# mjq11302010044/TATT

Hardware: AMD Instinct MI355X
Metric: LR images/s (train fwd+bwd+clip+Adam) at 16x64->32x128 (higher is better)
Workload: dtype fp32 (split-bf16 MFMA operands in conv3 / conv3-wgrad / conv9 / tokgemm / gru-wgrad / query-GRU recurrence and dW_hh / TP-layer backward)

## Files before the change

include/tatt_hip.h:

```cpp
#ifndef TATT_HIP_H
#define TATT_HIP_H

#ifdef __cplusplus
extern "C" {
#endif

typedef struct ihipStream_t* hipStream_t;


int tatt_gemm(const float* A, long sam, long sak, const float* A2, long sa2m, long sa2k, int K1,
              const float* B, long sbk, long sbn, const float* bias, float* C, long scm, long scn,
              int M, int N, int K, int Z, long bsA, long bsA2, long bsB, long bsC, long bsBias,
              float alpha, float beta, int act, int splitk, float* ws, float* rowsum, hipStream_t st);

int tatt_conv2d_fwd(const float* x, long xsn, long xsh, long xsw, long xsc, const float* wpacked,
                    const float* bias, float* y, long ldy, int Bn, int H, int W, int Cin, int Cout,
                    int KH, int KW, int act, float beta, int splitk, float* ws, hipStream_t st);

int tatt_conv2d_fwd_partials(const float* x, long xsn, long xsh, long xsw, long xsc, const float* wpacked, int Bn, int H,
                             int W, int Cin, int Cout, int KH, int KW, int splitk, float* ws, int* splits, hipStream_t st);

int tatt_conv2d_wgrad(const float* x, long xsn, long xsh, long xsw, long xsc, const float* dy,
                      long lddy, float* dw_oihw, int Bn, int H, int W, int Cin, int Cout, int KH,
                      int KW, float beta, int splitk, float* ws, hipStream_t st);

int tatt_repack_conv_weight(const float* w_oihw, float* out, int Cout, int Cin, int KH, int KW,
                            int mode, hipStream_t st);
int tatt_repack_words(int Cout, int Cin, int KH, int KW, int mode);
int tatt_repack_conv_weight_batch(const float* const* ws, float* const* outs, const int* dims, int n, hipStream_t st);

int tatt_gru_wgrad_sb(const float* dgi, const float* dgh, const float* x, const float* xb, const float* hprev,
                      float* ws1, float* ws2, int M, int G, hipStream_t st);

int tatt_splitk_reduce(const float* partial, float* C, int M, int N, int S, int remap_cin, int remap_taps,
                       float beta, float* vec, int vec_len, hipStream_t st);
int tatt_reduce_defer(int on, hipStream_t st);
int tatt_reduce_flush(hipStream_t st);

int tatt_conv3_c64_fwd_t(const float* x, const float* wt, const float* bias, float* y, int B, int H, int W, int Cin,
                         int Cout, int act, float beta, hipStream_t st);
int tatt_conv3_c64_fwd_ws16(const float* x, const float* wl, const float* bias, float* y, int B, int H, int W,
                            int Cout, int act, float beta, hipStream_t st);
int tatt_conv3_c64_fwd_ws16_bn(const float* x, const float* wl, const float* bias, float* y, int B, int H, int W,
                               int Cout, int act, float beta, const float* in_scale, const float* in_shift, int in_act,
                               double* stats, hipStream_t st);
int tatt_conv3_c64_fwd_sb(const float* x, int cin_total, int ci0, const float* wl, const float* bias, float* y, int B, int H,
                          int W, int Cout, int act, float beta, const float* in_scale, const float* in_shift, int in_act,
                          double* stats, hipStream_t st);
int tatt_conv3_c64_dgrad_bn_sb(const float* x, const float* x2, const float* in_scale, const float* in_scale2,
                               const float* in_shift, const float* wl, float* y, int B, int H, int W, const float* ep_x,
                               const float* ep_mean, const float* ep_rstd, const float* ep_gamma, const float* ep_beta,
                               int ep_act, double* stats, hipStream_t st);
int tatt_conv3_sb_generation(int gen);
int tatt_conv3_sb_packing(int B, int H, int W, int cin_total, int Cout, int act, int ep_act);
int tatt_conv3_sb_route(int B, int H, int W, int cin_total, int Cout, int act, int ep_act);
int tatt_conv3_c64_wgrad_partial(const float* x, const float* dy, float* part, float* pdb, int B, int H, int W,
                                 int Cin, int Cout, int G, hipStream_t st);
int tatt_conv3_c64_wgrad_partial_sb(const float* x, const float* dy, float* part, float* pdb, int B, int H, int W,
                                    int Cin, int Cout, int G, hipStream_t st);
int tatt_conv3_wgrad_sb_generation(int gen);
int tatt_conv3_wgrad_sb_route(int B, int H, int W, int Cin, int Cout);

int tatt_conv9_c64_to_c4(const float* x, const float* wpacked, const float* bias, float* y, int B, int H, int W,
                         int C, hipStream_t st);
int tatt_conv9_c64_to_c4_mfma(const float* x, const float* wt, const float* bias, float* y, int B, int H, int W,
                              hipStream_t st);
int tatt_conv9_c64_to_c4_sb(const float* x, const float* wt, const float* bias, float* y, int B, int H, int W,
                            hipStream_t st);
int tatt_conv9_c4_to_c64(const float* in, const float* wp, const float* bias, float* out, int B, int H, int W, int act,
                         hipStream_t st);
int tatt_conv9_c4_to_c64_sb(const float* in, const float* wp, const float* bias, float* out, int B, int H, int W, int act,
                            hipStream_t st);
int tatt_conv9_c64_c4_wgrad(const float* x, const float* dy, float* dw, float* part, int B, int H, int W,
                            hipStream_t st);
int tatt_conv9_c4_c64_wgrad(const float* x, const float* dy, float* dw, float* part, int B, int H, int W,
                            hipStream_t st);
int tatt_conv9_c64_c4_wgrad_sb(const float* x, const float* dy, float* dw, float* part, int B, int H, int W,
                               hipStream_t st);
int tatt_conv9_c4_c64_wgrad_sb(const float* x, const float* dy, float* dw, float* part, int B, int H, int W,
                               hipStream_t st);


int tatt_colsum(const float* X, long ld, int M, int C, float* out, float scale, float beta,
                double* ws, hipStream_t st);

int tatt_bn_stats(const float* X, long ld, int M, int C, float eps, float momentum, float* mean,
                  float* rstd, float* running_mean, float* running_var, double* ws, hipStream_t st);
int tatt_bn_stats_finish(const double* part, int G, int C, int M, float eps, float momentum, const float* gamma,
                         const float* beta, float* mean, float* rstd, float* running_mean, float* running_var, float* scale,
                         float* shift, hipStream_t st);
int tatt_bn_rstd(const float* var, float* rstd, int C, float eps, hipStream_t st);
int tatt_bn_apply(const float* X, long ldx, float* Y, long ldy, int M, int C, const float* mean,
                  const float* rstd, const float* gamma, const float* beta, int act, hipStream_t st);
int tatt_bn_bwd(const float* X, long ldx, const float* dY, long lddy, float* dX, long lddx, int M, int C,
                const float* mean, const float* rstd, const float* gamma, const float* beta, int act,
                int training, float* dgamma, float* dbeta, float* sums, double* ws, hipStream_t st);
int tatt_bn_bwd_groups(int M);
int tatt_bn_bwd_partials(const float* X, long ldx, const float* dY, long lddy, int M, int C, const float* mean,
                         const float* rstd, const float* gamma, const float* beta, int act, double* part, hipStream_t st);
int tatt_bn_bwd_finish(const double* part, int G, int C, int M, const float* mean, const float* rstd, const float* gamma,
                       float* dgamma, float* dbeta, float* coef, hipStream_t st);
int tatt_bn_bwd_affine(const float* X, const float* dU, float* dX, int M, int C, const float* coef, hipStream_t st);

int tatt_ln_fwd(const float* A, const float* Bres, float* Y, float* stats, int M, int C,
                const float* gamma, const float* beta, float eps, int mode, float pdrop,
                const unsigned long long* seed, unsigned site, hipStream_t st);
int tatt_ln_bwd(const float* A, const float* Bres, const float* dY, const float* stats, float* dX, float* dB, int M,
                int C, const float* gamma, float* dgamma, float* dbeta, float* part, double* ws, float eps, int mode,
                float pdrop, const unsigned long long* seed, unsigned site, hipStream_t st);


int tatt_prelu_fwd(const float* x, float* y, const float* alpha, long n, hipStream_t st);
int tatt_prelu_bwd(const float* x, const float* dy, float* dx, const float* alpha, long n, float* part,
                   hipStream_t st);
int tatt_act_fwd(const float* x, float* y, long n, int act, hipStream_t st);
int tatt_act_bwd(const float* ref, const float* dy, float* dx, long n, int act, int from_output,
                 hipStream_t st);
int tatt_axpby(const float* a, const float* b, float* y, float alpha, float beta, long n, hipStream_t st);
int tatt_add_n(const float* const* srcs, int n, float* y, long numel, hipStream_t st);
int tatt_add_rowbcast(const float* a, const float* b, float* y, long rows, int C, long period,
                      hipStream_t st);
int tatt_pixel_shuffle_fwd(const float* in, float* out, int B, int H, int W, int C, int act,
                           hipStream_t st);
int tatt_pixel_shuffle_bwd(const float* in, const float* dout, float* din, int B, int H, int W, int C,
                           int act, hipStream_t st);
int tatt_maxpool_fwd(const float* in, float* out, int B, int H, int W, int C, int kh, int kw, int sh, int sw,
                     int ph, int pw, hipStream_t st);
int tatt_maxpool_bwd(const float* in, const float* dout, float* din, int B, int H, int W, int C, int kh,
                     int kw, int sh, int sw, int ph, int pw, hipStream_t st);
int tatt_dropout(const float* x, float* y, long n, float p, const unsigned long long* seed, unsigned site,
                 hipStream_t st);
int tatt_bump_seed(unsigned long long* seed, unsigned long long* snap, hipStream_t st);
int tatt_stamp(unsigned long long* out, hipStream_t st);
int tatt_copy4d(const float* src, float* dst, int n0, int n1, int n2, int n3, long s0, long s1, long s2,
                long s3, long d0, long d1, long d2, long d3, float beta, hipStream_t st);


int tatt_l2norm(const float* g, long n, float* out, double* ws, hipStream_t st);
int tatt_adam_step(float* p, const float* g, float* m, float* v, long n, float lr, float b1, float b2,
                   float eps, const float* gnorm, float max_norm, float gscale, const long long* step,
                   hipStream_t st);


int tatt_gru32_fwd(const float* gi, const float* whh_f, const float* bhh_f, const float* whh_r,
// ... 293 lines not shown
```

tatt_amd/csrc/conv3.hip:

```cpp
#include "common.h"
#include <mutex>
#include <stdlib.h>
#include <type_traits>

#define C3_PX 64
#define C3_HW 66

struct Conv3P {
    const float* x; const float* w; const float* bias; float* y;
    int B, H, W, Cin, Cout, act;
    float beta;
    const float* in_scale; const float* in_shift; int in_act;
    double* stats;
};
template <int CK>
struct C5 {
    static constexpr int XP = CK + 4;
    static constexpr int HALO = 3 * C3_HW * XP;
    static constexpr int WT = 64 * XP;
    static constexpr int LDS = (2 * HALO + 2 * WT) * 4;
    static constexpr int Q4 = CK / 4;
    static constexpr int SLICE = 22 * Q4;
    static constexpr int WF4 = 64 * Q4;
};
// ... 239 lines not shown
        acc[1] = (f32x4){0.f, 0.f, 0.f, 0.f};
        f32x4 va[3][2];
        f32x4 hq = (f32x4){0.f, 0.f, 0.f, 0.f};
#define W16_AOFF(l, m) ((((l) >> 2) / 3 * C3_HW + ((l) >> 2) % 3 + 16 * (m)) * W16_XP + 16 * ((l) & 3))
#define W16_LD(l) va[(l) % 3][0] = *reinterpret_cast<const f32x4*>(Xs + W16_AOFF(l, 0)); \
                  va[(l) % 3][1] = *reinterpret_cast<const f32x4*>(Xs + W16_AOFF(l, 1));
        W16_LD(0) W16_LD(1)
#pragma unroll
        for (int l = 0; l < 36; ++l) {
            if (l % 5 == 0 && has_next) hq = halo_load(nn, nh, nw0, t + 512 * (l / 5));
            if (l + 2 < 36) { W16_LD(l + 2) }
            __builtin_amdgcn_sched_barrier(0);
#pragma unroll
            for (int u = 0; u < 4; ++u) {
                acc[0] = __builtin_amdgcn_mfma_f32_16x16x4f32(va[l % 3][0][u], wq[l][u], acc[0], 0, 0, 0);
                acc[1] = __builtin_amdgcn_mfma_f32_16x16x4f32(va[l % 3][1][u], wq[l][u], acc[1], 0, 0, 0);
            }
            __builtin_amdgcn_sched_barrier(0);
            if (l % 5 == 4 && has_next) halo_store(XsN, t + 512 * (l / 5), hq);
        }
        {
            const long rowbase = ((long)n * p.H + h) * p.W + w0 + pxh * 32 + 4 * (lane >> 4);
#pragma unroll
            for (int m = 0; m < 2; ++m)
#pragma unroll
                for (int r = 0; r < 4; ++r) {
                    float* dst = p.y + (rowbase + 16 * m + r) * p.Cout + co0 + (lane & 15);
                    float v = acc[m][r] + bj;
                    if (p.beta != 0.f) v += p.beta * *dst;
                    v = apply_act(v, p.act);
                    *dst = v;
                    st_s += v; st_q += v * v;
                }
        }
        if (!has_next) break;
        __syncthreads();
        pt = npt_next; n = nn; h = nh; w0 = nw0;
        xbuf ^= 1;
    }
    if (p.stats) {
        st_s += __shfl_xor(st_s, 16, 64); st_s += __shfl_xor(st_s, 32, 64);
        st_q += __shfl_xor(st_q, 16, 64); st_q += __shfl_xor(st_q, 32, 64);
        if (lane < 16) { st_red[pxh][0][cq * 16 + lane] = st_s; st_red[pxh][1][cq * 16 + lane] = st_q; }
        __syncthreads();
        if (t < 128) p.stats[(long)blockIdx.x * 128 + t] = (double)st_red[0][t >> 6][t & 63] + (double)st_red[1][t >> 6][t & 63];
    }
}

TATT_API int tatt_conv3_c64_fwd_ws16_bn(const float* x, const float* wl, const float* bias, float* y, int B, int H, int W,
                                        int Cout, int act, float beta, const float* in_scale, const float* in_shift, int in_act,
                                        double* stats, hipStream_t st);
TATT_API int tatt_conv3_c64_fwd_ws16(const float* x, const float* wl, const float* bias, float* y, int B, int H, int W,
                                     int Cout, int act, float beta, hipStream_t st) {
    return tatt_conv3_c64_fwd_ws16_bn(x, wl, bias, y, B, H, W, Cout, act, beta, nullptr, nullptr, 0, nullptr, st);
}
TATT_API int tatt_conv3_c64_fwd_ws16_bn(const float* x, const float* wl, const float* bias, float* y, int B, int H, int W,
                                        int Cout, int act, float beta, const float* in_scale, const float* in_shift, int in_act,
                                        double* stats, hipStream_t st) {
    if (Cout % 64 || W % C3_PX) return 1;
    if (stats && (Cout != 64 || act != ACT_NONE || beta != 0.f)) return 2;
    if (in_scale && (!in_shift || in_act == ACT_TANH)) return 3;
    Conv3P p = {x, wl, bias, y, B, H, W, 64, Cout, act, beta, in_scale, in_shift, in_act, stats};
    static TattPerDevice attr_once;
    tatt_per_device(attr_once, [&] {
        (void)hipFuncSetAttribute(reinterpret_cast<const void*>(conv3_c64_ws16_kernel), hipFuncAttributeMaxDynamicSharedMemorySize, W16_LDS);
    });
    const int cob = Cout / 64, npt = B * H * (W / C3_PX);
    int per = 256 / cob;
    if (per > npt) per = npt;
    hipLaunchKernelGGL(conv3_c64_ws16_kernel, dim3(per * cob), dim3(512), W16_LDS, st, p);
    return LAUNCH_CHECK();
}

typedef __bf16 bf16x8 __attribute__((ext_vector_type(8)));
typedef __bf16 bf16x2 __attribute__((ext_vector_type(2)));
typedef float f32x2 __attribute__((ext_vector_type(2)));
#define SB_PW 40
#define SB_IMG (3 * C3_HW * SB_PW)
#define SB_LDS (4 * SB_IMG * 4)
struct Conv3SB {
    Conv3P c; int cin_total, ci0;
    const float* x2; const float* in_scale2;
    const float* ep_x; const float* ep_mean; const float* ep_rstd; const float* ep_gamma; const float* ep_beta; int ep_act;
};
__device__ __forceinline__ void sb_split(f32x4 v, uint2& hi, uint2& lo) {
    const bf16x2 h0 = __builtin_convertvector((f32x2){v[0], v[1]}, bf16x2), h1 = __builtin_convertvector((f32x2){v[2], v[3]}, bf16x2);
    const unsigned u0 = __builtin_bit_cast(unsigned, h0), u1 = __builtin_bit_cast(unsigned, h1);
    const float r0 = v[0] - __builtin_bit_cast(float, u0 << 16), r1 = v[1] - __builtin_bit_cast(float, u0 & 0xffff0000u);
    const float r2 = v[2] - __builtin_bit_cast(float, u1 << 16), r3 = v[3] - __builtin_bit_cast(float, u1 & 0xffff0000u);
    const bf16x2 l0 = __builtin_convertvector((f32x2){r0, r1}, bf16x2), l1 = __builtin_convertvector((f32x2){r2, r3}, bf16x2);
    hi = make_uint2(u0, u1);
    lo = make_uint2(__builtin_bit_cast(unsigned, l0), __builtin_bit_cast(unsigned, l1));
}
template <bool IN2, bool EPBN>
__global__ __launch_bounds__(512, 1) void conv3_c64_sb_kernel(Conv3SB q) {
    const Conv3P& p = q.c;
    extern __shared__ __attribute__((aligned(16))) unsigned smem_u[];
    const int t = threadIdx.x, lane = t & 63, wave = t >> 6;
    const int cq = wave & 3, pxh = wave >> 2;
    const int segs = p.W / C3_PX, cob = p.Cout / 64;
    const int npt = p.B * p.H * segs;
    const int stride = gridDim.x / cob;
    int cb = blockIdx.x % cob, pt = blockIdx.x / cob;
    if (gridDim.x % 8 == 0 && 8 % cob == 0 && stride % (8 / cob) == 0) {
        const int x = blockIdx.x & 7, m = blockIdx.x >> 3, xg = 8 / cob;
        cb = x % cob;
        pt = (x / cob) * (stride / xg) + m;
    }
    __shared__ float st_red[2][2][64];
    if (pt >= npt) {
        if (p.stats && t < 128) p.stats[(long)blockIdx.x * 128 + t] = 0.0;
        return;
    }
    const int co0 = cb * 64 + cq * 16;
    f32x4 isc = (f32x4){1.f, 1.f, 1.f, 1.f}, ish = (f32x4){0.f, 0.f, 0.f, 0.f};
    if (p.in_scale) {
        isc = *reinterpret_cast<const f32x4*>(p.in_scale + 4 * (t & 15));
        ish = *reinterpret_cast<const f32x4*>(p.in_shift + 4 * (t & 15));
    }
    f32x4 isc2 = (f32x4){0.f, 0.f, 0.f, 0.f};
    if (IN2) isc2 = *reinterpret_cast<const f32x4*>(q.in_scale2 + 4 * (t & 15));
    float ep_mu = 0.f, ep_rs = 0.f, ep_g = 0.f, ep_b = 0.f;
    if (EPBN) {
        const int c = co0 + (lane & 15);
        ep_mu = q.ep_mean[c]; ep_rs = q.ep_rstd[c]; ep_g = q.ep_gamma[c]; ep_b = q.ep_beta[c];
    }
    float st_s = 0.f, st_q = 0.f;
    f32x4 wq[36];
    {
        const f32x4* wsrc = reinterpret_cast<const f32x4*>(p.w) + (long)(cb * 4 + cq) * 36 * 64 + lane;
#pragma unroll
        for (int k = 0; k < 36; ++k) wq[k] = wsrc[k * 64];
    }
    auto decode = [&](int tile, int& n, int& h, int& w0) {
        const int seg = tile % segs; tile /= segs;
        h = tile % p.H; n = tile / p.H; w0 = seg * C3_PX;
    };
    auto halo_load = [&](int n, int h, int w0, int idx) -> f32x4 {
        const int pix = idx >> 4, r = pix / C3_HW, px = pix - r * C3_HW;
        const int hh = h + r - 1, ww = w0 + px - 1;
        f32x4 v = (f32x4){0.f, 0.f, 0.f, 0.f};
        if (idx < 3 * C3_HW * 16 && hh >= 0 && hh < p.H && ww >= 0 && ww < p.W) {
            v = *reinterpret_cast<const f32x4*>(p.x + (((long)n * p.H + hh) * p.W + ww) * q.cin_total + q.ci0 + 4 * (idx & 15));
            if (IN2) {
                const f32x4 v2 = *reinterpret_cast<const f32x4*>(q.x2 + (((long)n * p.H + hh) * p.W + ww) * 64 + 4 * (idx & 15));
#pragma unroll
                for (int e = 0; e < 4; ++e) v[e] = fmaf(v[e], isc[e], fmaf(v2[e], isc2[e], ish[e]));
            } else if (p.in_scale) {
#pragma unroll
                for (int e = 0; e < 4; ++e) {
                    const float u = fmaf(v[e], isc[e], ish[e]);
                    v[e] = p.in_act == ACT_MISH ? mish_f(u) : (p.in_act == ACT_RELU ? fmaxf(u, 0.f) : u);
                }
            }
        }
        return v;
    };
    auto halo_store = [&](unsigned* Xs, int idx, f32x4 v) {
        if (idx < 3 * C3_HW * 16) {
            uint2 hi, lo;
            sb_split(v, hi, lo);
            unsigned* d = Xs + (idx >> 4) * SB_PW + 2 * (idx & 15);
            *reinterpret_cast<uint2*>(d) = hi;
            *reinterpret_cast<uint2*>(d + SB_IMG) = lo;
        }
    };
    int n, h, w0;
    decode(pt, n, h, w0);
    {
        f32x4 hp[7];
#pragma unroll
        for (int k = 0; k < 7; ++k) hp[k] = halo_load(n, h, w0, t + 512 * k);
#pragma unroll
        for (int k = 0; k < 7; ++k) halo_store(smem_u, t + 512 * k, hp[k]);
    }
// ... 282 lines not shown
        unsigned nnorg, nnte;
        decode(pt + 2 * stride, nnorg, nnte);
#pragma unroll
        for (int st = 0; st < 18; ++st) {
            if (st + 1 < 18) { S3_LD(st + 1) }
            if (FIRST && st % 2 == 0 && st / 2 + 3 < 9) w_issue(st / 2 + 3);
            __builtin_amdgcn_sched_barrier(0);
            const bf16x8 wh = __builtin_bit_cast(bf16x8, wq[2 * st]), wl = __builtin_bit_cast(bf16x8, wq[2 * st + 1]);
            const bf16x8 b0h = __builtin_bit_cast(bf16x8, vb[st % 2][0]), b0l = __builtin_bit_cast(bf16x8, vb[st % 2][1]);
            const bf16x8 b1h = __builtin_bit_cast(bf16x8, vb[st % 2][2]), b1l = __builtin_bit_cast(bf16x8, vb[st % 2][3]);
            accM[0] = __builtin_amdgcn_mfma_f32_32x32x16_bf16(wh, b0h, accM[0], 0, 0, 0);
            accM[1] = __builtin_amdgcn_mfma_f32_32x32x16_bf16(wh, b1h, accM[1], 0, 0, 0);
            accC[0] = __builtin_amdgcn_mfma_f32_32x32x16_bf16(wl, b0h, accC[0], 0, 0, 0);
            accC[1] = __builtin_amdgcn_mfma_f32_32x32x16_bf16(wl, b1h, accC[1], 0, 0, 0);
            accC[0] = __builtin_amdgcn_mfma_f32_32x32x16_bf16(wh, b0l, accC[0], 0, 0, 0);
            accC[1] = __builtin_amdgcn_mfma_f32_32x32x16_bf16(wh, b1l, accC[1], 0, 0, 0);
            if (st % 2 == 1 && st / 2 < S3_NIT) {
                halo_put(imgN, nte, st / 2);
                halo_issue1(nnorg, nnte, had_next && pt + 2 * stride < npt, st / 2);
                S3_INTERLEAVE(INMODE == 1 ? 14 : 8)
            }
            if (st % 4 == 2 && st / 4 < S3_NEP) { epilogue(epi_pending, st / 4); S3_INTERLEAVE(8) }
            if (st % 4 == 0 && st > 0 && st / 4 - 1 < S3_NEP) epi_request(org, st / 4 - 1);
            __builtin_amdgcn_sched_barrier(0);
        }
#if S2_STAMP
        { const unsigned long long now = __builtin_amdgcn_s_memtime();
          if (tix == 0) ts[3] = now; else if (tix == 1) ts[6] = now; else if (tix == 2) ts[9] = now; }
#endif
        has_next = had_next && pt + 2 * stride < npt;
        {
            unsigned* xw = XCH + xbuf * S2_XCH + (kh * 64 + lj) * S2_XP + 32 * coh + 4 * kb;
#pragma unroll
            for (int pp = 0; pp < 2; ++pp)
#pragma unroll
                for (int g = 0; g < 4; ++g) {
                    f32x4 v;
#pragma unroll
                    for (int r = 0; r < 4; ++r) v[r] = accM[pp][4 * g + r] + accC[pp][4 * g + r];
                    *reinterpret_cast<f32x4*>(xw + 32 * pp * S2_XP + 8 * g) = v;
                }
        }
        eorg = org; ebuf = xbuf; epi_pending = true;
#if S2_STAMP
        { const unsigned long long now = __builtin_amdgcn_s_memtime();
          if (tix == 0) ts[4] = now; else if (tix == 1) ts[7] = now; else if (tix == 2) ts[10] = now; }
        ++tix;
#endif
        __syncthreads();
        if (had_next) { pt += stride; org = norg; te = nte; norg = nnorg; nte = nnte; xbuf ^= 1; }
    };
    tile_body(std::true_type{});
    while (had_next) tile_body(std::false_type{});
    S2_STAMP_AT(11)
#pragma unroll
    for (int e = 0; e < S3_NEP; ++e) epilogue(true, e);
    S2_STAMP_AT(12)
#if S2_STAMP
    ts[31] = wall_clock64();
    if (lane == 0 && sbuf) {
#pragma unroll
        for (int i = 0; i < 32; ++i) sbuf[(blockIdx.x * 8 + wave) * 32 + i] = ts[i];
    }
#endif
    if (p.stats) {
#pragma unroll
        for (int r = 0; r < 4; ++r) {
            st_s[r] += __shfl_xor(st_s[r], 16, 64); st_s[r] += __shfl_xor(st_s[r], 32, 64);
            st_q[r] += __shfl_xor(st_q[r], 16, 64); st_q[r] += __shfl_xor(st_q[r], 32, 64);
        }
        if (lane < 16) {
#pragma unroll
            for (int r = 0; r < 4; ++r) { st_red[wave][0][ec4 + r] = st_s[r]; st_red[wave][1][ec4 + r] = st_q[r]; }
        }
        __syncthreads();
        if (t < 128) {
            double a = 0.0;
#pragma unroll
            for (int w = 0; w < 4; ++w) a += (double)st_red[w][t >> 6][t & 63];
            p.stats[(long)blockIdx.x * 128 + t] = a;
        }
    }
}
template <int INMODE, bool EPBN>
__global__ __launch_bounds__(512, 2) void conv3_c64_sb4_kernel(Conv3SB q) {
    const Conv3P& p = q.c;
    extern __shared__ __attribute__((aligned(16))) unsigned smem_u[];
    unsigned* const XCH = smem_u + 4 * S3_IMG;
    const unsigned t = threadIdx.x, lane = t & 63, wave = t >> 6;
    const unsigned W = p.W, H = p.H, tws = (W + 15) / 16, ths = H / 4, cob = p.Cout / 64;
    const unsigned npt = p.B * ths * tws;
    const unsigned stride = gridDim.x / cob;
    unsigned cb = blockIdx.x % cob, pt = blockIdx.x / cob;
    if (gridDim.x % 8 == 0 && 8 % cob == 0 && stride % (8 / cob) == 0) {
        const unsigned x = blockIdx.x & 7, m = blockIdx.x >> 3, xg = 8 / cob;
        cb = x % cob;
        pt = (x / cob) * (stride / xg) + m;
    }
    __shared__ float st_red[4][2][64];
    __shared__ __attribute__((aligned(16))) float cst[7][64];
    __shared__ __attribute__((aligned(16))) float cbias[64];
    if (pt >= npt) {
        if (p.stats && t < 128) p.stats[(long)blockIdx.x * 128 + t] = 0.0;
        return;
    }
    const unsigned ntile = (npt - pt + stride - 1) / stride;
    auto decode = [&](unsigned tile, unsigned& org, unsigned& te) {
        const unsigned tw = tile % tws; tile /= tws;
        const unsigned th = tile % ths, n = tile / ths;
        org = (n * H + th * 4) * W + tw * 16;
        const unsigned cin = min(18u, W - tw * 16 + 1);
        te = (th == 0 ? 1u : 0u) | (th == ths - 1 ? 2u : 0u) | (tw == 0 ? 4u : 0u) | (cin << 8);
    };
    if (wave >= 4) {
        const unsigned h = t - 256;
        const unsigned npix = p.B * H * W;
        const __amdgpu_buffer_rsrc_t rs_x = __builtin_amdgcn_make_buffer_rsrc(const_cast<float*>(p.x), 0, npix * q.cin_total * 4, 0x00020000);
        const __amdgpu_buffer_rsrc_t rs_x2 = __builtin_amdgcn_make_buffer_rsrc(const_cast<float*>(INMODE == 2 ? q.x2 : p.x), 0, npix * 256, 0x00020000);
        const __amdgpu_buffer_rsrc_t rs_y = __builtin_amdgcn_make_buffer_rsrc(p.y, 0, npix * p.Cout * 4, 0x00020000);
        const __amdgpu_buffer_rsrc_t rs_e = __builtin_amdgcn_make_buffer_rsrc(const_cast<float*>(EPBN ? q.ep_x : p.y), 0, npix * (EPBN ? 64 : p.Cout) * 4, 0x00020000);
        const bool in_relu = p.in_act == ACT_RELU;
        const unsigned xps = q.cin_total * 4, yps = p.Cout * 4, eps_ = EPBN ? 256u : yps;
        unsigned boff[S3_NIT], poff[S3_NIT], edge[2] = {0, 0}, colk[2] = {0, 0};
#pragma unroll
        for (int k = 0; k < S3_NIT; ++k) {
            const unsigned pix = (h >> 4) + 16 * k, r = pix / S2_HW, c = pix - r * S2_HW;
            boff[k] = (unsigned)(((int)r - 1) * (int)W + (int)c - 1) * xps + (q.ci0 + 4 * (h & 15)) * 4;
            poff[k] = r * S3_RP + c * SB_PW + 2 * (h & 15);
            edge[k >> 2] |= ((r == 0 ? 1u : 0u) | (r == 5 ? 2u : 0u) | (c == 0 ? 4u : 0u) | (pix >= S2_NPX ? 8u : 0u)) << (8 * (k & 3));
            colk[k >> 2] |= c << (8 * (k & 3));
        }
        auto outside = [&](int k, unsigned te) -> bool {
            return (((edge[k >> 2] >> (8 * (k & 3))) & (te | 8u) & 15u) != 0) || (((colk[k >> 2] >> (8 * (k & 3))) & 255u) >= (te >> 8));
        };
        f32x4 hp[S3_NIT], hp2[S3_NIT];
        auto halo_issue = [&](unsigned tile, bool valid) {
            unsigned org, te;
            decode(tile, org, te);
#if S2_DEBUG
            if (s2_wrep & 4) valid = false;
#endif
#pragma unroll
            for (int k = 0; k < S3_NIT; ++k) {
                const unsigned a = (org * xps + boff[k]) | (outside(k, te) ? S2_OOB : (valid ? 0u : S2_OOB));
                hp[k] = s2_ld(rs_x, a);
                if (INMODE == 2) hp2[k] = s2_ld(rs_x2, a);
            }
        };
        auto halo_put = [&](unsigned* img, unsigned tile) {
            unsigned org, te;
            decode(tile, org, te);
            f32x4 isc, ish, isc2;
            if (INMODE != 0) { isc = *reinterpret_cast<const f32x4*>(&cst[0][4 * (h & 15)]); ish = *reinterpret_cast<const f32x4*>(&cst[1][4 * (h & 15)]); }
            if (INMODE == 2) isc2 = *reinterpret_cast<const f32x4*>(&cst[2][4 * (h & 15)]);
#pragma unroll
            for (int k = 0; k < S3_NIT; ++k) {
                const bool ok = !outside(k, te);
                f32x4 v = hp[k];
                if (INMODE == 2) {
#pragma unroll
                    for (int e = 0; e < 4; ++e) v[e] = fmaf(v[e], isc[e], fmaf(hp2[k][e], isc2[e], ish[e]));
                } else if (INMODE == 1) {
#pragma unroll
                    for (int e = 0; e < 4; ++e) v[e] = mish_f(fmaf(v[e], isc[e], ish[e]));
                } else if (INMODE == 3) {
#pragma unroll
                    for (int e = 0; e < 4; ++e) {
                        const float u = fmaf(v[e], isc[e], ish[e]);
                        v[e] = in_relu ? fmaxf(u, 0.f) : u;
                    }
                }
                if (INMODE != 0) {
#pragma unroll
                    for (int e = 0; e < 4; ++e) v[e] = ok ? v[e] : 0.f;
                }
                if (k < S3_NIT - 1 || h < S2_NPX * 16 - 256 * (S3_NIT - 1)) {
                    uint2 hi, lo;
                    sb_split(v, hi, lo);
                    unsigned* d = img + poff[k];
                    *reinterpret_cast<uint2*>(d) = hi;
                    *reinterpret_cast<uint2*>(d + S3_IMG) = lo;
                }
            }
        };
        halo_issue(pt, true);
        if (h < 64) {
            cbias[h] = p.bias ? p.bias[cb * 64 + h] : 0.f;
            if (INMODE != 0) { cst[0][h] = p.in_scale[h]; cst[1][h] = p.in_shift[h]; }
            if (INMODE == 2) cst[2][h] = q.in_scale2[h];
            if (EPBN) { cst[3][h] = q.ep_mean[h]; cst[4][h] = q.ep_rstd[h]; cst[5][h] = q.ep_gamma[h]; cst[6][h] = q.ep_beta[h]; }
        }
        __syncthreads();
        halo_put(smem_u, pt);
        halo_issue(pt + stride, ntile > 1);
        __syncthreads();
        const bool use_beta = p.beta != 0.f, out_relu = p.act == ACT_RELU;
        const bool ep_mish = q.ep_act == ACT_MISH, ep_relu = q.ep_act == ACT_RELU;
        const unsigned ecol = h >> 4, ec4 = 4 * (h & 15);
        f32x4 epx[S3_NEP], st_s = (f32x4){0.f, 0.f, 0.f, 0.f}, st_q = st_s;
        auto epi_request = [&](unsigned tile) {
            unsigned org, te;
            decode(tile, org, te);
            const bool in_map = ecol + 1 < (te >> 8);
#pragma unroll
            for (int e = 0; e < S3_NEP; ++e)
                epx[e] = s2_ld(rs_e, ((org + e * W + ecol) * eps_ + (cb * 64 + ec4) * 4) | (((EPBN || use_beta) && in_map) ? 0u : S2_OOB));
        };
        auto epilogue = [&](unsigned tile, unsigned xb) {
            unsigned org, te;
            decode(tile, org, te);
            const f32x4 bj = *reinterpret_cast<const f32x4*>(&cbias[ec4]);
            const bool in_map = ecol + 1 < (te >> 8);
            f32x4 ep_mu, ep_rs, ep_g, ep_b;
            if (EPBN) {
                ep_mu = *reinterpret_cast<const f32x4*>(&cst[3][ec4]); ep_rs = *reinterpret_cast<const f32x4*>(&cst[4][ec4]);
                ep_g = *reinterpret_cast<const f32x4*>(&cst[5][ec4]); ep_b = *reinterpret_cast<const f32x4*>(&cst[6][ec4]);
            }
#pragma unroll
            for (int e = 0; e < S3_NEP; ++e) {
                const unsigned* X = XCH + xb * S2_XCH + ((h >> 4) + 16 * e) * S2_XP + ec4;
                const f32x4 v0 = *reinterpret_cast<const f32x4*>(X), v1 = *reinterpret_cast<const f32x4*>(X + 64 * S2_XP);
                f32x4 v;
#pragma unroll
                for (int r = 0; r < 4; ++r) {
                    v[r] = (v0[r] + v1[r]) + bj[r];
                    if (EPBN) {
                        const float xh = (epx[e][r] - ep_mu[r]) * ep_rs[r], u = fmaf(ep_g[r], xh, ep_b[r]);
                        const float g = ep_mish ? mish_grad_f(u) : 1.f;
                        v[r] *= ep_relu ? (u > 0.f ? 1.f : 0.f) : g;
                        v[r] = in_map ? v[r] : 0.f;
                        st_s[r] += v[r]; st_q[r] += v[r] * xh;
                    } else {
                        v[r] = fmaf(p.beta, epx[e][r], v[r]);
                        v[r] = out_relu ? fmaxf(v[r], 0.f) : v[r];
                        v[r] = in_map ? v[r] : 0.f;
                        st_s[r] += v[r]; st_q[r] += v[r] * v[r];
                    }
                }
#if S2_DEBUG
                if (s2_wrep & 8) continue;
#endif
                __builtin_amdgcn_raw_buffer_store_b128(__builtin_bit_cast(u32x4_s2, v), rs_y, ((org + e * W + ecol) * yps + (cb * 64 + ec4) * 4) | (in_map ? 0u : S2_OOB), 0, 0);
            }
        };
        for (unsigned i = 0; i < ntile; ++i) {
            const unsigned tile = pt + i * stride;
#if S2_DEBUG
            if (s2_wrep & 1) { __syncthreads(); continue; }
#endif
#if S2_DEBUG
            if (!(s2_wrep & 32))
#endif
            if (i > 0) epilogue(tile - stride, (i - 1) & 1);
#if S2_DEBUG
            if (!(s2_wrep & 16))
#endif
            if (i + 1 < ntile) halo_put(smem_u + ((i + 1) & 1) * 2 * S3_IMG, tile + stride);
            halo_issue(tile + 2 * stride, i + 2 < ntile);
            epi_request(tile);
            __syncthreads();
        }
        epilogue(pt + (ntile - 1) * stride, (ntile - 1) & 1);
        if (p.stats) {
#pragma unroll
            for (int r = 0; r < 4; ++r) {
                st_s[r] += __shfl_xor(st_s[r], 16, 64); st_s[r] += __shfl_xor(st_s[r], 32, 64);
                st_q[r] += __shfl_xor(st_q[r], 16, 64); st_q[r] += __shfl_xor(st_q[r], 32, 64);
            }
            if (lane < 16) {
#pragma unroll
                for (int r = 0; r < 4; ++r) { st_red[wave - 4][0][ec4 + r] = st_s[r]; st_red[wave - 4][1][ec4 + r] = st_q[r]; }
            }
        }
        __syncthreads();
        if (p.stats && h < 128) {
            double a = 0.0;
#pragma unroll
            for (int w = 0; w < 4; ++w) a += (double)st_red[w][h >> 6][h & 63];
            p.stats[(long)blockIdx.x * 128 + h] = a;
        }
        return;
    }
    const unsigned coh = wave & 1, kh = wave >> 1, lj = lane & 31, kb = lane >> 5;
    f32x4 wq[36];
    {
        const f32x4* const wsrc = reinterpret_cast<const f32x4*>(p.w) + (cb * 2 + coh) * 72 * 64 + lane;
#pragma unroll
        for (int tap = 0; tap < 9; ++tap)
#pragma unroll
            for (int f = 0; f < 4; ++f) wq[4 * tap + f] = wsrc[((tap * 2 + kh) * 4 + f) * 64];
    }
    const unsigned bbase = (lj >> 4) * S3_RP + (lj & 15) * SB_PW + 16 * kh + 4 * kb;
    __syncthreads();
    __syncthreads();
    for (unsigned i = 0; i < ntile; ++i) {
#if S2_DEBUG
        if (s2_wrep & 2) { __syncthreads(); continue; }
#endif
        const unsigned* Xs = smem_u + (i & 1) * 2 * S3_IMG + bbase;
        f32x16_s3 acc[2];
#pragma unroll
        for (int pp = 0; pp < 2; ++pp)
#pragma unroll
            for (int v = 0; v < 16; ++v) acc[pp][v] = 0.f;
        f32x4 vb[2][4];
        S3_LD(0)
#pragma unroll
        for (int st = 0; st < 18; ++st) {
            if (st + 1 < 18) { S3_LD(st + 1) }
            __builtin_amdgcn_sched_barrier(0);
            const bf16x8 wh = __builtin_bit_cast(bf16x8, wq[2 * st]), wl = __builtin_bit_cast(bf16x8, wq[2 * st + 1]);
            const bf16x8 b0h = __builtin_bit_cast(bf16x8, vb[st % 2][0]), b0l = __builtin_bit_cast(bf16x8, vb[st % 2][1]);
            const bf16x8 b1h = __builtin_bit_cast(bf16x8, vb[st % 2][2]), b1l = __builtin_bit_cast(bf16x8, vb[st % 2][3]);
            acc[0] = __builtin_amdgcn_mfma_f32_32x32x16_bf16(wh, b0h, acc[0], 0, 0, 0);
            acc[1] = __builtin_amdgcn_mfma_f32_32x32x16_bf16(wh, b1h, acc[1], 0, 0, 0);
            acc[0] = __builtin_amdgcn_mfma_f32_32x32x16_bf16(wl, b0h, acc[0], 0, 0, 0);
            acc[1] = __builtin_amdgcn_mfma_f32_32x32x16_bf16(wl, b1h, acc[1], 0, 0, 0);
            acc[0] = __builtin_amdgcn_mfma_f32_32x32x16_bf16(wh, b0l, acc[0], 0, 0, 0);
            acc[1] = __builtin_amdgcn_mfma_f32_32x32x16_bf16(wh, b1l, acc[1], 0, 0, 0);
            __builtin_amdgcn_sched_barrier(0);
        }
        unsigned* xw = XCH + (i & 1) * S2_XCH + (kh * 64 + lj) * S2_XP + 32 * coh + 4 * kb;
#pragma unroll
        for (int pp = 0; pp < 2; ++pp)
#pragma unroll
            for (int g = 0; g < 4; ++g) {
                f32x4 v;
#pragma unroll
                for (int r = 0; r < 4; ++r) v[r] = acc[pp][4 * g + r];
                *reinterpret_cast<f32x4*>(xw + 32 * pp * S2_XP + 8 * g) = v;
            }
        __syncthreads();
    }
    __syncthreads();
}
static int conv3_sb_generation = 4;
TATT_API int tatt_conv3_sb_generation(int gen) {
    const int old = conv3_sb_generation;
    if (gen == 1 || gen == 3 || gen == 4) conv3_sb_generation = gen;
    return old;
}
template <int INMODE, bool EPBN>
static void conv3_sb4_go(const Conv3SB& q, dim3 grid, hipStream_t st) {
    static TattPerDevice attr_once;
    tatt_per_device(attr_once, [&] {
        (void)hipFuncSetAttribute(reinterpret_cast<const void*>(conv3_c64_sb4_kernel<INMODE, EPBN>), hipFuncAttributeMaxDynamicSharedMemorySize, S3_LDS);
    });
    hipLaunchKernelGGL((conv3_c64_sb4_kernel<INMODE, EPBN>), grid, dim3(512), S3_LDS, st, q);
}
template <int INMODE, bool EPBN>
static void conv3_sb3_go(const Conv3SB& q, dim3 grid, hipStream_t st) {
    static TattPerDevice attr_once;
    tatt_per_device(attr_once, [&] {
        (void)hipFuncSetAttribute(reinterpret_cast<const void*>(conv3_c64_sb3_kernel<INMODE, EPBN>), hipFuncAttributeMaxDynamicSharedMemorySize, S3_LDS);
    });
    hipLaunchKernelGGL((conv3_c64_sb3_kernel<INMODE, EPBN>), grid, dim3(256), S3_LDS, st, q);
}
static int conv3_sb_pick(int B, int H, int W, int cin_total, int Cout, int act, int ep_act) {
    const long maxb = (long)B * H * W * (cin_total > Cout ? cin_total : Cout) * 4;
    if (conv3_sb_generation < 3 || H % 4 || maxb >= 0x7fffffffL || ep_act == ACT_TANH) return 1;
    if (conv3_sb_generation == 4 && (act == ACT_NONE || (act == ACT_RELU && ep_act == ACT_NONE))) return 4;
    return (conv3_sb_generation == 3 && W % 16 == 0 && act == ACT_NONE) ? 3 : 1;
}
TATT_API int tatt_conv3_sb_packing(int B, int H, int W, int cin_total, int Cout, int act, int ep_act) {
    return conv3_sb_pick(B, H, W, cin_total, Cout, act, ep_act) >= 3 ? 14 : 10;
}
TATT_API int tatt_conv3_sb_route(int B, int H, int W, int cin_total, int Cout, int act, int ep_act) {
    const int pick = conv3_sb_pick(B, H, W, cin_total, Cout, act, ep_act);
    return pick == 1 && W % C3_PX ? 0 : pick;
}
static int conv3_sb_launch(const Conv3SB& q, hipStream_t st) {
    const Conv3P& p = q.c;
    const int pick = conv3_sb_pick(p.B, p.H, p.W, q.cin_total, p.Cout, p.act, q.ep_act);
    if (pick >= 3) {
        const int cob = p.Cout / 64, npt = p.B * (p.H / 4) * ((p.W + 15) / 16);
        int per = 256 / cob;
        if (per > npt) per = npt;
        const dim3 grid(per * cob);
        const bool ep = q.ep_x != nullptr;
        const int inmode = q.x2 ? 2 : (p.in_scale ? (p.in_act == ACT_MISH ? 1 : 3) : 0);
        if (pick == 4) {
            if (inmode == 2) { if (ep) conv3_sb4_go<2, true>(q, grid, st); else conv3_sb4_go<2, false>(q, grid, st); }
            else if (inmode == 1) { if (ep) conv3_sb4_go<1, true>(q, grid, st); else conv3_sb4_go<1, false>(q, grid, st); }
            else if (inmode == 3) { if (ep) conv3_sb4_go<3, true>(q, grid, st); else conv3_sb4_go<3, false>(q, grid, st); }
            else { if (ep) conv3_sb4_go<0, true>(q, grid, st); else conv3_sb4_go<0, false>(q, grid, st); }
            return LAUNCH_CHECK();
        }
        if (pick == 3) {
            if (inmode == 2) { if (ep) conv3_sb3_go<2, true>(q, grid, st); else conv3_sb3_go<2, false>(q, grid, st); }
            else if (inmode == 1) { if (ep) conv3_sb3_go<1, true>(q, grid, st); else conv3_sb3_go<1, false>(q, grid, st); }
            else if (inmode == 3) { if (ep) conv3_sb3_go<3, true>(q, grid, st); else conv3_sb3_go<3, false>(q, grid, st); }
            else { if (ep) conv3_sb3_go<0, true>(q, grid, st); else conv3_sb3_go<0, false>(q, grid, st); }
            return LAUNCH_CHECK();
        }
        return LAUNCH_CHECK();
    }
    if (p.W % C3_PX) return 1;
    static TattPerDevice attr_once;
    tatt_per_device(attr_once, [&] {
        (void)hipFuncSetAttribute(reinterpret_cast<const void*>(conv3_c64_sb_kernel<false, false>), hipFuncAttributeMaxDynamicSharedMemorySize, SB_LDS);
        (void)hipFuncSetAttribute(reinterpret_cast<const void*>(conv3_c64_sb_kernel<true, false>), hipFuncAttributeMaxDynamicSharedMemorySize, SB_LDS);
        (void)hipFuncSetAttribute(reinterpret_cast<const void*>(conv3_c64_sb_kernel<false, true>), hipFuncAttributeMaxDynamicSharedMemorySize, SB_LDS);
        (void)hipFuncSetAttribute(reinterpret_cast<const void*>(conv3_c64_sb_kernel<true, true>), hipFuncAttributeMaxDynamicSharedMemorySize, SB_LDS);
    });
    const int cob = p.Cout / 64, npt = p.B * p.H * (p.W / C3_PX);
    int per = 256 / cob;
    if (per > npt) per = npt;
    const dim3 grid(per * cob), block(512);
    const bool in2 = q.x2 != nullptr, ep = q.ep_x != nullptr;
    if (in2 && ep) hipLaunchKernelGGL((conv3_c64_sb_kernel<true, true>), grid, block, SB_LDS, st, q);
    else if (in2) hipLaunchKernelGGL((conv3_c64_sb_kernel<true, false>), grid, block, SB_LDS, st, q);
    else if (ep) hipLaunchKernelGGL((conv3_c64_sb_kernel<false, true>), grid, block, SB_LDS, st, q);
    else hipLaunchKernelGGL((conv3_c64_sb_kernel<false, false>), grid, block, SB_LDS, st, q);
    return LAUNCH_CHECK();
}
TATT_API int tatt_conv3_c64_fwd_sb(const float* x, int cin_total, int ci0, const float* wl, const float* bias, float* y, int B, int H,
                                   int W, int Cout, int act, float beta, const float* in_scale, const float* in_shift, int in_act,
                                   double* stats, hipStream_t st) {
    if (Cout % 64 || cin_total % 4 || ci0 % 4 || ci0 + 64 > cin_total) return 1;
    if (stats && (Cout != 64 || act != ACT_NONE || beta != 0.f)) return 2;
    if (in_scale && (!in_shift || in_act == ACT_TANH)) return 3;
    Conv3SB q = {{x, wl, bias, y, B, H, W, 64, Cout, act, beta, in_scale, in_shift, in_act, stats}, cin_total, ci0,
                 nullptr, nullptr, nullptr, nullptr, nullptr, nullptr, nullptr, 0};
    return conv3_sb_launch(q, st);
}
TATT_API int tatt_conv3_c64_dgrad_bn_sb(const float* x, const float* x2, const float* in_scale, const float* in_scale2,
                                        const float* in_shift, const float* wl, float* y, int B, int H, int W, const float* ep_x,
                                        const float* ep_mean, const float* ep_rstd, const float* ep_gamma, const float* ep_beta,
                                        int ep_act, double* stats, hipStream_t st) {
    if (x2 && (!in_scale || !in_scale2 || !in_shift)) return 2;
    if (ep_x && (!ep_mean || !ep_rstd || !ep_gamma || !ep_beta || !stats)) return 3;
    if (!ep_x && stats) return 4;
    Conv3SB q = {{x, wl, nullptr, y, B, H, W, 64, 64, ACT_NONE, 0.f, x2 ? in_scale : nullptr, x2 ? in_shift : nullptr, ACT_NONE, stats}, 64, 0,
                 x2, in_scale2, ep_x, ep_mean, ep_rstd, ep_gamma, ep_beta, ep_act};
    return conv3_sb_launch(q, st);
}

struct Conv3WP {
    const float* x; const float* dy; float* part;
    int B, H, W, Cin, Cout, nseg;
    float* pdb;
};
#define WG_HALO (3 * C3_HW * 64)
#define WG_BUF (WG_HALO + 64 * 64)
#define C3_WG_LDS (2 * WG_BUF * 4)
#define WG_F4 (WG_BUF / 4)

template <int T0, int NT>
__device__ __forceinline__ void wgrad_segment(f32x16 (&acc)[5], const float* __restrict__ acol, const float* __restrict__ bcol,
                                              const Conv3WP& p, bool has_next, int nn, int nh, int nw0, int ci0, int co0,
                                              float* __restrict__ nbuf, int t, float& dbacc) {
    auto fetch = [&](int idx) -> f32x4 {
        f32x4 v = (f32x4){0.f, 0.f, 0.f, 0.f};
        if (idx < WG_HALO / 4) {
            const int c4 = idx & 15, pp = idx >> 4;
            const int r = pp / C3_HW, px = pp - r * C3_HW;
            const int hh = nh + r - 1, ww = nw0 + px - 1;
            if (hh >= 0 && hh < p.H && ww >= 0 && ww < p.W)
                v = *reinterpret_cast<const f32x4*>(p.x + (((long)nn * p.H + hh) * p.W + ww) * p.Cin + ci0 + 4 * c4);
        } else if (idx < WG_F4) {
            const int j = idx - WG_HALO / 4, c4 = j & 15, px = j >> 4;
            v = *reinterpret_cast<const f32x4*>(p.dy + (((long)nn * p.H + nh) * p.W + nw0 + px) * p.Cout + co0 + 4 * c4);
        }
        return v;
    };
    float wa[2][NT], wb[2];
    f32x4 pf = (f32x4){0.f, 0.f, 0.f, 0.f};
#define C3W_LOAD(buf, k)                                                                   \
    wb[buf] = bcol[(k) * 64];                                                              \
    _Pragma("unroll") for (int tp = 0; tp < NT; ++tp)                                      \
        wa[buf][tp] = acol[(((T0 + tp) / 3) * C3_HW + (k) + ((T0 + tp) % 3)) * 64];
    C3W_LOAD(0, 0)
    __builtin_amdgcn_sched_barrier(0);
#pragma unroll
    for (int k = 0; k < 64; k += 2) {
        const int cur = (k >> 1) & 1;
        if (k + 2 < 64) { C3W_LOAD(cur ^ 1, k + 2) }
        if (has_next && k % 6 == 0 && k / 6 < 9) pf = fetch(t + 512 * (k / 6));
        __builtin_amdgcn_sched_barrier(0);
#pragma unroll
        for (int tp = 0; tp < NT; ++tp)
            acc[tp] = __builtin_amdgcn_mfma_f32_32x32x2f32(wa[cur][tp], wb[cur], acc[tp], 0, 0, 0);
        if (T0 == 0) dbacc += wb[cur];
        __builtin_amdgcn_sched_barrier(0);
        if (has_next && k % 6 == 4 && k / 6 < 9) {
            const int idx = t + 512 * (k / 6);
            if (idx < WG_F4) *reinterpret_cast<f32x4*>(nbuf + 4 * idx) = pf;
        }
    }
#undef C3W_LOAD
}

#define WS_TP 36
#define WS_TT (32 * WS_TP)
__global__ __launch_bounds__(512, 1) void conv3_c64_wgrad_kernel(Conv3WP p) {
    extern __shared__ __attribute__((aligned(16))) float smem[];
    const int t = threadIdx.x, lane = t & 63, wave = t >> 6;
    const int qi = wave & 1, qo = (wave >> 1) & 1, tg = wave >> 2;
    const int cib = blockIdx.y % (p.Cin / 64), cob = blockIdx.y / (p.Cin / 64);
    const int ci0 = cib * 64, co0 = cob * 64;
    const int segs = p.W / C3_PX;
    f32x16 acc[5];
#pragma unroll
    for (int a = 0; a < 5; ++a)
#pragma unroll
        for (int i = 0; i < 16; ++i) acc[a][i] = 0.f;
    auto decode = [&](int s, int& n, int& h, int& w0) {
        const int seg = s % segs; s /= segs;
        h = s % p.H; n = s / p.H; w0 = seg * C3_PX;
    };
    float dbacc = 0.f;
    int s = blockIdx.x;
    if (s < p.nseg) {
        int n, h, w0;
        decode(s, n, h, w0);
        {
            f32x4 v[9];
// ... 81 lines not shown
```

tatt_amd/csrc/conv3w.hip:

```cpp
#include "common.h"
#include <mutex>

typedef __bf16 cw_bf16x8 __attribute__((ext_vector_type(8)));
typedef __bf16 cw_bf16x2 __attribute__((ext_vector_type(2)));
typedef float cw_f32x2 __attribute__((ext_vector_type(2)));

#define CW_PX 64
#define CW_HW 66
#define CW_CP 66
#define CW_HALO (3 * CW_HW * CW_CP)
#define CW_IMG (CW_HALO + CW_PX * CW_CP)
#define CW_NFRAG 32
#define CW_FRAGS (CW_NFRAG * 2 * 64 * 4)
#define CW_LDS ((CW_IMG + CW_FRAGS) * 4)
#define CW_F4 ((3 * CW_HW * 64 + CW_PX * 64) / 4)

struct Conv3WSP {
    const float* x; const float* dy; float* part;
    int B, H, W, Cin, Cout, nseg;
    float* pdb;
};

__device__ __forceinline__ void cw_split(const float* v, cw_bf16x8& hi, cw_bf16x8& lo) {
#pragma unroll
    for (int e = 0; e < 8; e += 2) {
        const cw_f32x2 a = (cw_f32x2){v[e], v[e + 1]};
        const cw_bf16x2 h = __builtin_convertvector(a, cw_bf16x2);
        const cw_bf16x2 l = __builtin_convertvector(a - __builtin_convertvector(h, cw_f32x2), cw_bf16x2);
        hi[e] = h[0]; hi[e + 1] = h[1];
        lo[e] = l[0]; lo[e + 1] = l[1];
    }
}
__device__ __forceinline__ void cw_put(float* F, int f, int lane, const cw_bf16x8& hi, const cw_bf16x8& lo) {
    *reinterpret_cast<f32x4*>(F + ((f * 2 + 0) * 64 + lane) * 4) = __builtin_bit_cast(f32x4, hi);
    *reinterpret_cast<f32x4*>(F + ((f * 2 + 1) * 64 + lane) * 4) = __builtin_bit_cast(f32x4, lo);
}
__device__ __forceinline__ cw_bf16x8 cw_get(const float* F, int f, int hl, int lane) {
    return __builtin_bit_cast(cw_bf16x8, *reinterpret_cast<const f32x4*>(F + ((f * 2 + hl) * 64 + lane) * 4));
}
__device__ __forceinline__ f32x4 cw_mma3(const cw_bf16x8& ah, const cw_bf16x8& al, const cw_bf16x8& bh, const cw_bf16x8& bl, f32x4 c) {
    c = __builtin_amdgcn_mfma_f32_16x16x32_bf16(ah, bh, c, 0, 0, 0);
    c = __builtin_amdgcn_mfma_f32_16x16x32_bf16(ah, bl, c, 0, 0, 0);
    return __builtin_amdgcn_mfma_f32_16x16x32_bf16(al, bh, c, 0, 0, 0);
}

__global__ __launch_bounds__(512, 1) void conv3_c64_wgrad_sb_kernel(Conv3WSP p) {
    extern __shared__ __attribute__((aligned(16))) float cw_smem[];
    float* const IMG = cw_smem;
    float* const F = cw_smem + CW_IMG;
    const int t = threadIdx.x, lane = t & 63, wave = t >> 6, li = lane & 15, kq = lane >> 4;
    const int ct = wave & 3, cg = wave >> 2;
    const int cib = blockIdx.y % (p.Cin / 64), cob = blockIdx.y / (p.Cin / 64);
    const int ci0 = cib * 64, co0 = cob * 64;
    const int segs = p.W / CW_PX;
    const bool want_db = p.pdb != nullptr && cib == 0 && ct == 0;
    f32x4 acc[9][2], accdb[2];
#pragma unroll
    for (int a = 0; a < 9; ++a) { acc[a][0] = (f32x4){0.f, 0.f, 0.f, 0.f}; acc[a][1] = acc[a][0]; }
    accdb[0] = (f32x4){0.f, 0.f, 0.f, 0.f}; accdb[1] = accdb[0];
    cw_bf16x8 ones;
#pragma unroll
    for (int e = 0; e < 8; ++e) ones[e] = (__bf16)1.0f;
    const int per = (p.nseg + (int)gridDim.x - 1) / (int)gridDim.x;
    const int s_beg = blockIdx.x * per, s_end = min(p.nseg, s_beg + per);
    f32x4 pre[9];
    auto seg_of = [&](int s, int& n, int& h, int& w0) { h = s % p.H; s /= p.H; w0 = (s % segs) * CW_PX; n = s / segs; };
    auto fetch = [&](int s) {
        int n, h, w0;
        seg_of(s, n, h, w0);
        const bool fresh = s == s_beg || h == 0;
#pragma unroll
        for (int r = 0; r < 9; ++r) {
            const int idx = t + 512 * r;
            f32x4 u = (f32x4){0.f, 0.f, 0.f, 0.f};
            if (idx < 3 * CW_HW * 16) {
                const int c4 = idx & 15, pp = idx >> 4;
                const int rr = pp / CW_HW, px = pp - rr * CW_HW;
                const int hh = h + rr - 1, ww = w0 + px - 1;
                if ((fresh || rr == 2) && hh >= 0 && hh < p.H && ww >= 0 && ww < p.W)
                    u = *reinterpret_cast<const f32x4*>(p.x + (((long)n * p.H + hh) * p.W + ww) * p.Cin + ci0 + 4 * c4);
            } else if (idx < CW_F4) {
                const int j = idx - 3 * CW_HW * 16, c4 = j & 15, px = j >> 4;
                u = *reinterpret_cast<const f32x4*>(p.dy + (((long)n * p.H + h) * p.W + w0 + px) * p.Cout + co0 + 4 * c4);
            }
            pre[r] = u;
        }
    };
    auto stash = [&](int s) {
        int n, h, w0;
        seg_of(s, n, h, w0);
        const bool fresh = s == s_beg || h == 0;
#pragma unroll
        for (int r = 0; r < 9; ++r) {
            const int idx = t + 512 * r;
            if (idx < CW_F4) {
                float* d;
                if (idx < 3 * CW_HW * 16) {
                    const int pp = idx >> 4, rr = pp / CW_HW, px = pp - rr * CW_HW;
                    if (!(fresh || rr == 2)) continue;
                    d = IMG + (((h + rr + 2) % 3) * CW_HW + px) * CW_CP + 4 * (idx & 15);
                } else { const int j = idx - 3 * CW_HW * 16; d = IMG + CW_HALO + (j >> 4) * CW_CP + 4 * (j & 15); }
                *reinterpret_cast<float2*>(d) = make_float2(pre[r][0], pre[r][1]);
                *reinterpret_cast<float2*>(d + 2) = make_float2(pre[r][2], pre[r][3]);
// ... 13 lines not shown
            {
                const int xt = (wave >> 1) & 3, ks = wave & 1;
                const float* col = IMG + ((((hrow + ky + 2) % 3) * CW_HW + 32 * ks + 8 * kq) * CW_CP) + 16 * xt + li;
                float v[10];
#pragma unroll
                for (int e = 0; e < 10; ++e) v[e] = col[e * CW_CP];
#pragma unroll
                for (int kx = 0; kx < 3; ++kx) {
                    cw_bf16x8 hi, lo;
                    cw_split(v + kx, hi, lo);
                    cw_put(F, (kx * 4 + xt) * 2 + ks, lane, hi, lo);
                }
                if (ky == 0) {
                    const float* dcol = IMG + CW_HALO + (32 * ks + 8 * kq) * CW_CP + 16 * (wave >> 1) + li;
                    float w8[8];
#pragma unroll
                    for (int e = 0; e < 8; ++e) w8[e] = dcol[e * CW_CP];
                    cw_bf16x8 hi, lo;
                    cw_split(w8, hi, lo);
                    cw_put(F, 24 + (wave >> 1) * 2 + ks, lane, hi, lo);
                }
            }
            __syncthreads();
            if (ky == 0) {
#pragma unroll
                for (int c = 0; c < 2; ++c)
#pragma unroll
                    for (int ks = 0; ks < 2; ++ks) {
                        dh[c][ks] = cw_get(F, 24 + (2 * cg + c) * 2 + ks, 0, lane);
                        dl[c][ks] = cw_get(F, 24 + (2 * cg + c) * 2 + ks, 1, lane);
                        if (want_db) {
                            accdb[c] = __builtin_amdgcn_mfma_f32_16x16x32_bf16(ones, dh[c][ks], accdb[c], 0, 0, 0);
                            accdb[c] = __builtin_amdgcn_mfma_f32_16x16x32_bf16(ones, dl[c][ks], accdb[c], 0, 0, 0);
                        }
                    }
            }
#pragma unroll
            for (int kx = 0; kx < 3; ++kx)
#pragma unroll
                for (int ks = 0; ks < 2; ++ks) {
                    const cw_bf16x8 ah = cw_get(F, (kx * 4 + ct) * 2 + ks, 0, lane), al = cw_get(F, (kx * 4 + ct) * 2 + ks, 1, lane);
#pragma unroll
                    for (int c = 0; c < 2; ++c) acc[ky * 3 + kx][c] = cw_mma3(ah, al, dh[c][ks], dl[c][ks], acc[ky * 3 + kx][c]);
                }
            __syncthreads();
        }
    }
    float* P = p.part + (long)blockIdx.x * 9 * p.Cin * p.Cout;
#pragma unroll
    for (int tap = 0; tap < 9; ++tap)
#pragma unroll
        for (int c = 0; c < 2; ++c)
#pragma unroll
            for (int r = 0; r < 4; ++r)
                P[((long)tap * p.Cin + ci0 + 16 * ct + 4 * kq + r) * p.Cout + co0 + 16 * (2 * cg + c) + li] = acc[tap][c][r];
    if (want_db && kq == 0) {
#pragma unroll
        for (int c = 0; c < 2; ++c) p.pdb[(long)blockIdx.x * p.Cout + co0 + 16 * (2 * cg + c) + li] = accdb[c][0];
    }
}

typedef __attribute__((__vector_size__(4 * sizeof(__bf16)))) __bf16 cw_bf16x4_t;
typedef __attribute__((address_space(3))) cw_bf16x4_t* cw_lds_b64;
typedef float cw_f32x16 __attribute__((ext_vector_type(16)));
typedef unsigned cw_u32x4 __attribute__((ext_vector_type(4)));
#define W2_PB 192
#define W2_XIMG (108 * W2_PB)
#define W2_DIMG (64 * W2_PB)
#define W2_BUF (2 * W2_XIMG + 2 * W2_DIMG)
#define W2_LDS (2 * W2_BUF)
#define W2_OOB 0x80000000u
__device__ __forceinline__ cw_bf16x8 w2_tr(const char* p0, int off) {
    const cw_bf16x4_t a = __builtin_amdgcn_ds_read_tr16_b64_v4bf16((cw_lds_b64)(p0 + off));
    const cw_bf16x4_t b = __builtin_amdgcn_ds_read_tr16_b64_v4bf16((cw_lds_b64)(p0 + off + 4 * W2_PB));
    return __builtin_shufflevector(a, b, 0, 1, 2, 3, 4, 5, 6, 7);
}
__device__ __forceinline__ void w2_split_put(char* dst_hi, int lo_off, f32x4 v) {
    const cw_bf16x2 h0 = __builtin_convertvector((cw_f32x2){v[0], v[1]}, cw_bf16x2), h1 = __builtin_convertvector((cw_f32x2){v[2], v[3]}, cw_bf16x2);
    const cw_f32x2 r0 = (cw_f32x2){v[0], v[1]} - __builtin_convertvector(h0, cw_f32x2), r1 = (cw_f32x2){v[2], v[3]} - __builtin_convertvector(h1, cw_f32x2);
    const cw_bf16x2 l0 = __builtin_convertvector(r0, cw_bf16x2), l1 = __builtin_convertvector(r1, cw_bf16x2);
    *reinterpret_cast<uint2*>(dst_hi) = make_uint2(__builtin_bit_cast(unsigned, h0), __builtin_bit_cast(unsigned, h1));
    *reinterpret_cast<uint2*>(dst_hi + lo_off) = make_uint2(__builtin_bit_cast(unsigned, l0), __builtin_bit_cast(unsigned, l1));
}
__global__ __launch_bounds__(512, 2) void conv3_c64_wgrad_sb2_kernel(Conv3WSP p) {
    extern __shared__ __attribute__((aligned(16))) char w2_smem[];
    __shared__ float dbred[16][64];
    const unsigned t = threadIdx.x, lane = t & 63, wave = t >> 6;
    const unsigned cib = blockIdx.y % (p.Cin / 64), cob = blockIdx.y / (p.Cin / 64);
    const unsigned ci0 = cib * 64, co0 = cob * 64;
    const unsigned W = p.W, H = p.H, tws = (W + 15) / 16, ths = H / 4;
    const unsigned per = (p.nseg + gridDim.x - 1) / gridDim.x;
    const unsigned s_beg = blockIdx.x * per, s_end = min((unsigned)p.nseg, s_beg + per);
    const bool want_db = p.pdb != nullptr && cib == 0;
    auto decode = [&](unsigned tile, unsigned& org, unsigned& te) {
        const unsigned tw = tile % tws; tile /= tws;
        const unsigned th = tile % ths, n = tile / ths;
        org = (n * H + th * 4) * W + tw * 16;
        te = (th == 0 ? 1u : 0u) | (th == ths - 1 ? 2u : 0u) | (tw == 0 ? 4u : 0u) | (min(18u, W - tw * 16 + 1) << 8);
    };
    if (wave >= 4) {
        const unsigned h = t - 256, c4 = h & 15;
        const unsigned npix = p.B * H * W;
        const __amdgpu_buffer_rsrc_t rs_x = __builtin_amdgcn_make_buffer_rsrc(const_cast<float*>(p.x), 0, npix * p.Cin * 4, 0x00020000);
        const __amdgpu_buffer_rsrc_t rs_d = __builtin_amdgcn_make_buffer_rsrc(const_cast<float*>(p.dy), 0, npix * p.Cout * 4, 0x00020000);
        const unsigned xps = p.Cin * 4, dps = p.Cout * 4;
        unsigned xoff[7], xput[7], edge[2] = {0, 0}, colk[2] = {0, 0}, doff[4], dput[4];
#pragma unroll
        for (int k = 0; k < 7; ++k) {
            const unsigned pix = (h >> 4) + 16 * k, r = pix / 18, c = pix - r * 18;
            xoff[k] = (unsigned)(((int)r - 1) * (int)W + (int)c - 1) * xps + (ci0 + 4 * c4) * 4;
            xput[k] = pix * W2_PB + 8 * c4;
            edge[k >> 2] |= ((r == 0 ? 1u : 0u) | (r == 5 ? 2u : 0u) | (c == 0 ? 4u : 0u) | (pix >= 108 ? 8u : 0u)) << (8 * (k & 3));
            colk[k >> 2] |= c << (8 * (k & 3));
        }
#pragma unroll
        for (int k = 0; k < 4; ++k) {
            const unsigned pix = (h >> 4) + 16 * k;
            doff[k] = (k * W + (h >> 4)) * dps + (co0 + 4 * c4) * 4;
            dput[k] = 2 * W2_XIMG + pix * W2_PB + 8 * c4;
        }
        f32x4 hx[7], hd[4], dbacc = (f32x4){0.f, 0.f, 0.f, 0.f};
        auto issue = [&](unsigned tile, bool valid) {
            unsigned org, te;
            decode(tile, org, te);
            const unsigned inv = valid ? 0u : W2_OOB;
#pragma unroll
            for (int k = 0; k < 7; ++k) {
                const bool out = (((edge[k >> 2] >> (8 * (k & 3))) & (te | 8u) & 15u) != 0) || (((colk[k >> 2] >> (8 * (k & 3))) & 255u) >= (te >> 8));
                hx[k] = __builtin_bit_cast(f32x4, __builtin_amdgcn_raw_buffer_load_b128(rs_x, (org * xps + xoff[k]) | (out ? W2_OOB : inv), 0, 0));
            }
            const unsigned dinv = ((h >> 4) + 1 < (te >> 8)) ? inv : W2_OOB;
#pragma unroll
            for (int k = 0; k < 4; ++k)
                hd[k] = __builtin_bit_cast(f32x4, __builtin_amdgcn_raw_buffer_load_b128(rs_d, (org * dps + doff[k]) | dinv, 0, 0));
        };
        auto put = [&](char* buf) {
#pragma unroll
            for (int k = 0; k < 7; ++k)
                if (k < 6 || h < 1728 - 6 * 256) w2_split_put(buf + xput[k], W2_XIMG, hx[k]);
#pragma unroll
            for (int k = 0; k < 4; ++k) { w2_split_put(buf + dput[k], W2_DIMG, hd[k]); dbacc += hd[k]; }
        };
        if (s_beg < s_end) {
            issue(s_beg, true);
            put(w2_smem);
            issue(s_beg + 1, s_beg + 1 < s_end);
        }
        __syncthreads();
        for (unsigned s = s_beg; s < s_end; ++s) {
            if (s + 1 < s_end) {
                put(w2_smem + ((s + 1 - s_beg) & 1) * W2_BUF);
                issue(s + 2, s + 2 < s_end);
            }
            __syncthreads();
        }
        if (want_db) {
#pragma unroll
            for (int e = 0; e < 4; ++e) dbred[h >> 4][4 * c4 + e] = dbacc[e];
        }
        __syncthreads();
        if (want_db && h < 64) {
            float a = 0.f;
#pragma unroll
            for (int g = 0; g < 16; ++g) a += dbred[g][h];
            p.pdb[(long)blockIdx.x * p.Cout + co0 + h] = a;
        }
        return;
    }
    const unsigned cih = wave & 1, coh = wave >> 1, a16 = lane & 15, g16 = (lane >> 4) & 1, kb = lane >> 5;
    cw_f32x16 acc[9];
#pragma unroll
    for (int tp = 0; tp < 9; ++tp)
#pragma unroll
        for (int i = 0; i < 16; ++i) acc[tp][i] = 0.f;
    const unsigned la = (8 * kb + (a16 >> 2)) * W2_PB + (32 * cih + 16 * g16) * 2 + (a16 & 3) * 8;
    const unsigned lb = 2 * W2_XIMG + (8 * kb + (a16 >> 2)) * W2_PB + (32 * coh + 16 * g16) * 2 + (a16 & 3) * 8;
    __syncthreads();
    for (unsigned s = s_beg; s < s_end; ++s) {
        const char* buf = w2_smem + ((s - s_beg) & 1) * W2_BUF;
        const char* pa = buf + la;
        const char* pb = buf + lb;
#pragma unroll
        for (int r = 0; r < 4; ++r) {
            const cw_bf16x8 bh = w2_tr(pb, r * 16 * W2_PB), bl = w2_tr(pb, r * 16 * W2_PB + W2_DIMG);
#pragma unroll
            for (int ky = 0; ky < 3; ++ky) {
                cw_bf16x8 ah[3], al[3];
#pragma unroll
                for (int kx = 0; kx < 3; ++kx) {
                    ah[kx] = w2_tr(pa, ((r + ky) * 18 + kx) * W2_PB);
                    al[kx] = w2_tr(pa, ((r + ky) * 18 + kx) * W2_PB + W2_XIMG);
                }
#pragma unroll
                for (int kx = 0; kx < 3; ++kx) acc[ky * 3 + kx] = __builtin_amdgcn_mfma_f32_32x32x16_bf16(ah[kx], bh, acc[ky * 3 + kx], 0, 0, 0);
#pragma unroll
                for (int kx = 0; kx < 3; ++kx) acc[ky * 3 + kx] = __builtin_amdgcn_mfma_f32_32x32x16_bf16(ah[kx], bl, acc[ky * 3 + kx], 0, 0, 0);
#pragma unroll
                for (int kx = 0; kx < 3; ++kx) acc[ky * 3 + kx] = __builtin_amdgcn_mfma_f32_32x32x16_bf16(al[kx], bh, acc[ky * 3 + kx], 0, 0, 0);
            }
        }
        __syncthreads();
    }
    __syncthreads();
    float* P = p.part + (long)blockIdx.x * 9 * p.Cin * p.Cout;
    float* T = reinterpret_cast<float*>(w2_smem) + wave * (32 * 36);
#pragma unroll
    for (int tp = 0; tp < 9; ++tp) {
#pragma unroll
        for (int v = 0; v < 16; ++v) T[((v & 3) + 8 * (v >> 2) + 4 * kb) * 36 + (lane & 31)] = acc[tp][v];
        wave_lds_sync();
#pragma unroll
        for (int qd = 0; qd < 4; ++qd) {
            const int row = (lane >> 3) + 8 * qd, cq4 = lane & 7;
            const f32x4 v = *reinterpret_cast<const f32x4*>(T + row * 36 + 4 * cq4);
            *reinterpret_cast<f32x4*>(P + ((long)tp * p.Cin + ci0 + 32 * cih + row) * p.Cout + co0 + 32 * coh + 4 * cq4) = v;
        }
        wave_lds_sync();
    }
}
static int conv3_wgrad_sb_generation = 2;
TATT_API int tatt_conv3_wgrad_sb_generation(int gen) {
    const int old = conv3_wgrad_sb_generation;
    if (gen == 1 || gen == 2) conv3_wgrad_sb_generation = gen;
    return old;
}
static int conv3_wgrad_sb_pick(int B, int H, int W, int Cin, int Cout) {
    if (Cin % 64 || Cout % 64) return 0;
    const long maxb = (long)B * H * W * (Cin > Cout ? Cin : Cout) * 4;
    if (conv3_wgrad_sb_generation == 2 && H % 4 == 0 && maxb < 0x7fffffffL) return 2;
    return W % CW_PX ? 0 : 1;
}
TATT_API int tatt_conv3_wgrad_sb_route(int B, int H, int W, int Cin, int Cout) { return conv3_wgrad_sb_pick(B, H, W, Cin, Cout); }

TATT_API int tatt_conv3_c64_wgrad_partial_sb(const float* x, const float* dy, float* part, float* pdb, int B, int H, int W,
                                             int Cin, int Cout, int G, hipStream_t st) {
    const int pick = conv3_wgrad_sb_pick(B, H, W, Cin, Cout);
    if (pick == 0) return 1;
    if (pick == 2) {
        const int ntile = B * (H / 4) * ((W + 15) / 16);
        Conv3WSP p2 = {x, dy, part, B, H, W, Cin, Cout, ntile, pdb};
        static TattPerDevice attr2_once;
        tatt_per_device(attr2_once, [&] {
            (void)hipFuncSetAttribute(reinterpret_cast<const void*>(conv3_c64_wgrad_sb2_kernel), hipFuncAttributeMaxDynamicSharedMemorySize, W2_LDS);
        });
        hipLaunchKernelGGL(conv3_c64_wgrad_sb2_kernel, dim3(G, (Cin / 64) * (Cout / 64)), dim3(512), W2_LDS, st, p2);
        return LAUNCH_CHECK();
    }
    const int nseg = B * H * (W / CW_PX);
    Conv3WSP p = {x, dy, part, B, H, W, Cin, Cout, nseg, pdb};
    static TattPerDevice attr_once;
    tatt_per_device(attr_once, [&] {
        (void)hipFuncSetAttribute(reinterpret_cast<const void*>(conv3_c64_wgrad_sb_kernel), hipFuncAttributeMaxDynamicSharedMemorySize, CW_LDS);
    });
    hipLaunchKernelGGL(conv3_c64_wgrad_sb_kernel, dim3(G, (Cin / 64) * (Cout / 64)), dim3(512), CW_LDS, st, p);
    return LAUNCH_CHECK();
}
```

tatt_amd/csrc/gemm.hip:

```cpp
#include "common.h"
#include <mutex>
#include <unordered_map>
#include <stdlib.h>

#define BM 64
#define BN 64
#define KC 16
#define LDT 65

struct GemmP {
    const float* A; const float* A2; const float* B; const float* bias; float* C;
    int M, N, K, K1;
    long sam, sak, sa2m, sa2k, sbk, sbn, scm, scn;
    long bsA, bsA2, bsB, bsC, bsBias;
    float alpha, beta;
    int act;
    int splitk, chunks_per_split;
    float* partial;
    float* rowsum;
    int H, W, Cin, KH, KW, pad, HW, Wshift, HWshift, Cshift;
    long xsn, xsh, xsw, xsc;
};

__device__ __forceinline__ void decode_pixel(const GemmP& p, int pix, int& n, int& h, int& w) {
// ... 475 lines not shown
                *reinterpret_cast<f32x4*>(p.partial + ((long)(z * p.splitk + blockIdx.y) * p.M + i) * p.N + j) = v;
            } else {
                float* dst = p.C + (long)z * p.bsC + i * p.scm + j;
                f32x4 o = (f32x4){0.f, 0.f, 0.f, 0.f};
                if (p.beta != 0.f) o = *reinterpret_cast<const f32x4*>(dst);
#pragma unroll
                for (int e = 0; e < 4; ++e) v[e] = apply_act(p.alpha * (v[e] + b4[e]), p.act) + p.beta * o[e];
                *reinterpret_cast<f32x4*>(dst) = v;
            }
        }
        return;
    }
    const int j = n0 + (lane & 31);
    float* C = p.C + (long)z * p.bsC;
    const float bj = p.bias ? p.bias[(long)z * p.bsBias + j] : 0.f;
#pragma unroll
    for (int reg = 0; reg < 16; ++reg) {
        const long i = m0 + wave * 32 + (reg & 3) + 8 * (reg >> 2) + 4 * (lane >> 5);
        if (i >= p.M) continue;
        float v = apply_act(p.alpha * (acc[reg] + bj), p.act);
        const long off = i * p.scm + j * p.scn;
        if (p.beta != 0.f) v += p.beta * C[off];
        C[off] = v;
    }
}

static inline bool al16(const void* q) { return ((uintptr_t)q & 15) == 0; }
static int try_gemm_fast(const GemmP& p, int Z, hipStream_t st) {
    const bool narrow = (p.N & 63) == 32;
    if ((!narrow && (p.N & 63)) || (p.K & 15)) return -1;
    const bool akc = p.sak == 1, amc = p.sam == 1 && !akc;
    if ((p.M & (narrow ? 127 : 63)) && !akc) return -1;
    if (narrow && (p.A2 || p.rowsum)) return -1;
    const bool bkc = p.sbk == 1 && p.sbn != 1, bnc = p.sbn == 1;
    if (!(akc || amc) || !(bkc || bnc)) return -1;
    if (!al16(p.A) || !al16(p.B) || (p.bsA & 3) || (p.bsB & 3)) return -1;
    if (akc ? (p.sam & 3) : (p.sak & 3)) return -1;
    if (bkc ? (p.sbn & 3) : (p.sbk & 3)) return -1;
    const bool cat = p.A2 != nullptr;
    if (cat && (!akc || p.sa2k != 1 || (p.sa2m & 3) || (p.K1 & 15) || !al16(p.A2) || (p.bsA2 & 3))) return -1;
    if (p.rowsum && akc) return -1;
    if (p.splitk > 1 && !al16(p.partial)) return -1;
    const int cvec = (p.scn == 1 && !(p.scm & 3) && al16(p.C) && !(p.bsC & 3) && (!p.bias || (al16(p.bias) && !(p.bsBias & 3)))) ? 1 : 0;
    if (narrow) {
        dim3 grid32(cdiv(p.M, 128) * (p.N >> 5), p.splitk, Z);
        if (akc && bkc) hipLaunchKernelGGL((gemm_fast32_kernel<true, true>), grid32, dim3(256), 0, st, p, cvec);
        else if (akc) hipLaunchKernelGGL((gemm_fast32_kernel<true, false>), grid32, dim3(256), 0, st, p, cvec);
        else if (bkc) hipLaunchKernelGGL((gemm_fast32_kernel<false, true>), grid32, dim3(256), 0, st, p, cvec);
        else hipLaunchKernelGGL((gemm_fast32_kernel<false, false>), grid32, dim3(256), 0, st, p, cvec);
        return LAUNCH_CHECK();
    }
    dim3 grid(cdiv(p.M, 64) * (p.N >> 6), p.splitk, Z), block(256);
#define GF_LAUNCH(A_, B_, C_) hipLaunchKernelGGL((gemm_fast_kernel<A_, B_, C_, false>), grid, block, 0, st, p, cvec)
    if (cat) { if (bkc) GF_LAUNCH(true, true, true); else GF_LAUNCH(true, false, true); }
    else if (akc) { if (bkc) GF_LAUNCH(true, true, false); else GF_LAUNCH(true, false, false); }
    else { if (bkc) GF_LAUNCH(false, true, false); else GF_LAUNCH(false, false, false); }
#undef GF_LAUNCH
    return LAUNCH_CHECK();
}
static int try_wgrad_fast(const GemmP& p, hipStream_t st) {
    if ((p.N & 63) || (p.Cin & 63) || (p.K & 15) || p.xsc != 1 || p.sbn != 1 || (p.sbk & 3) || p.splitk < 2) return -1;
    if (!al16(p.A) || !al16(p.B) || !al16(p.partial) || (p.xsn & 3) || (p.xsh & 3) || (p.xsw & 3)) return -1;
    dim3 grid((p.M >> 6) * (p.N >> 6), p.splitk, 1), block(256);
    hipLaunchKernelGGL((gemm_fast_kernel<false, false, false, false, true>), grid, block, 0, st, p, 0);
    return LAUNCH_CHECK();
}
static int try_conv_fast(const GemmP& p, hipStream_t st) {
    if ((p.N & 63) || (p.Cin & 15) || p.xsc != 1 || p.sbn != 1 || (p.sbk & 3)) return -1;
    if (!al16(p.A) || !al16(p.B) || (p.xsn & 3) || (p.xsh & 3) || (p.xsw & 3)) return -1;
    if (p.splitk > 1 && !al16(p.partial)) return -1;
    const int cvec = (p.scn == 1 && !(p.scm & 3) && al16(p.C) && (!p.bias || al16(p.bias))) ? 1 : 0;
    dim3 grid(cdiv(p.M, 64) * (p.N >> 6), p.splitk, 1), block(256);
    hipLaunchKernelGGL((gemm_fast_kernel<true, false, false, true>), grid, block, 0, st, p, cvec);
    return LAUNCH_CHECK();
}

struct ReduceArgs {
    const float* partial; float* C; const float* bias; float* rowsum;
    long scm, scn, bsC, bsBias;
    int M, N, S, Z;
    float alpha, beta;
    int act, remap_cin, remap_taps, block0;
    int RM;
};
__device__ __forceinline__ void splitk_reduce_body(const ReduceArgs& a, long block) {
    __shared__ float sh[4][64];
    const float* __restrict__ partial = a.partial;
    float* __restrict__ C = a.C;
    const int M = a.M, N = a.N, S = a.S, Z = a.Z;
    const int tx = threadIdx.x & 63, ty = threadIdx.x >> 6;
    const long idx = block * 64 + tx;
    const long total = (long)Z * M * N;
    const long total64 = ((total + 63) / 64) * 64;
    if (a.rowsum && idx >= total64) {
        const long i2 = idx - total64;
        const int rm = a.RM > 0 ? a.RM : M;
        float r = 0.f;
        if (i2 < rm) for (int k = ty; k < S; k += 4) r += partial[(long)S * M * N + (long)k * rm + i2];
        sh[ty][tx] = r;
        __syncthreads();
        if (ty == 0 && i2 < rm) a.rowsum[i2] = a.alpha * ((sh[0][tx] + sh[1][tx]) + (sh[2][tx] + sh[3][tx]));
        return;
    }
    const bool ok = idx < total;
    int j = 0, i = 0, z = 0;
    float s = 0.f;
    if (ok) {
        j = idx % N;
        long rest = idx / N;
        i = rest % M;
        z = rest / M;
        const long step = (long)M * N;
        const float* pp = partial + ((long)z * S * M + i) * N + j;
        float a0 = 0.f, a1 = 0.f, a2 = 0.f, a3 = 0.f;
        int k = ty;
        for (; k + 12 < S; k += 16) {
            float v0 = pp[(long)k * step], v1 = pp[(long)(k + 4) * step], v2 = pp[(long)(k + 8) * step], v3 = pp[(long)(k + 12) * step];
            a0 += v0; a1 += v1; a2 += v2; a3 += v3;
        }
        for (; k < S; k += 4) a0 += pp[(long)k * step];
        s = (a0 + a1) + (a2 + a3);
    }
    sh[ty][tx] = s;
    __syncthreads();
    if (ty != 0 || !ok) return;
    s = (sh[0][tx] + sh[1][tx]) + (sh[2][tx] + sh[3][tx]);
    float bj = a.bias ? a.bias[(long)z * a.bsBias + j] : 0.f;
    float v = apply_act(a.alpha * (s + bj), a.act);
    long off;
    if (a.remap_cin > 0) {
        int tap = i / a.remap_cin, ci = i - tap * a.remap_cin;
        off = ((long)j * a.remap_cin + ci) * a.remap_taps + tap;
    } else {
        off = (long)z * a.bsC + i * a.scm + j * a.scn;
    }
    if (a.beta != 0.f) v += a.beta * C[off];
    C[off] = v;
}
__global__ __launch_bounds__(256) void splitk_reduce_kernel(ReduceArgs a) { splitk_reduce_body(a, blockIdx.x); }

#define REDUCE_MAX 36
struct ReduceTable { ReduceArgs e[REDUCE_MAX]; int n; };
__global__ __launch_bounds__(256) void splitk_reduce_batch_kernel(ReduceTable t) {
    int k = 0;
    while (k + 1 < t.n && (int)blockIdx.x >= t.e[k + 1].block0) ++k;
    splitk_reduce_body(t.e[k], (long)blockIdx.x - t.e[k].block0);
}
struct ReduceState { bool defer = false; int n = 0; ReduceArgs pending[REDUCE_MAX]; };
static std::mutex g_reduce_mu;
static std::unordered_map<hipStream_t, ReduceState> g_reduce_states;
static long reduce_blocks(const ReduceArgs& a) {
    long total = (long)a.Z * a.M * a.N;
    if (a.rowsum) total = (long)cdiv(total, 64) * 64 + (a.RM > 0 ? a.RM : a.M);
    return cdiv(total, 64);
}
static int reduce_flush_locked(ReduceState& rs, hipStream_t st) {
    if (rs.n == 0) return 0;
    ReduceTable t;
    t.n = rs.n;
    int blocks = 0;
    for (int k = 0; k < t.n; ++k) {
        t.e[k] = rs.pending[k];
        t.e[k].block0 = blocks;
        blocks += (int)reduce_blocks(t.e[k]);
    }
    rs.n = 0;
    hipLaunchKernelGGL(splitk_reduce_batch_kernel, dim3(blocks), dim3(256), 0, st, t);
    return LAUNCH_CHECK();
}
static int reduce_flush(hipStream_t st) {
    std::lock_guard<std::mutex> lock(g_reduce_mu);
    auto it = g_reduce_states.find(st);
    return it == g_reduce_states.end() ? 0 : reduce_flush_locked(it->second, st);
}
static int reduce_submit(const ReduceArgs& a, hipStream_t st) {
    std::lock_guard<std::mutex> lock(g_reduce_mu);
    auto it = g_reduce_states.find(st);
    if (it == g_reduce_states.end() || !it->second.defer || a.beta != 0.f) {
        if (it != g_reduce_states.end()) {
            int rc = reduce_flush_locked(it->second, st);
            if (rc) return rc;
        }
        hipLaunchKernelGGL(splitk_reduce_kernel, dim3((unsigned)reduce_blocks(a)), dim3(256), 0, st, a);
        return LAUNCH_CHECK();
    }
    ReduceState& rs = it->second;
    rs.pending[rs.n++] = a;
    return rs.n == REDUCE_MAX ? reduce_flush_locked(rs, st) : 0;
}
TATT_API int tatt_reduce_defer(int on, hipStream_t st) {
    std::lock_guard<std::mutex> lock(g_reduce_mu);
    if (on) { g_reduce_states[st].defer = true; return 0; }
    auto it = g_reduce_states.find(st);
    if (it == g_reduce_states.end()) return 0;
    const int rc = reduce_flush_locked(it->second, st);
    g_reduce_states.erase(it);
    return rc;
}
TATT_API int tatt_reduce_flush(hipStream_t st) { return reduce_flush(st); }

static int ilog2_or_neg(int v) {
    if (v <= 0 || (v & (v - 1))) return -1;
    int s = 0;
    while ((1 << s) < v) ++s;
    return s;
}

template <int AMODE, int KCT>
static int launch_gemm(const GemmP& p, int Z, bool ak, bool bk, hipStream_t st) {
    dim3 grid(cdiv(p.M, BM) * cdiv(p.N, BN), p.splitk, Z), block(256);
    if (AMODE == 3) {
        if (bk) hipLaunchKernelGGL((gemm_mfma_kernel<3, 1, 1, 16>), grid, block, 0, st, p);
        else    hipLaunchKernelGGL((gemm_mfma_kernel<3, 1, 0, 16>), grid, block, 0, st, p);
    } else if (AMODE == 4) {
        if (bk) hipLaunchKernelGGL((gemm_mfma_kernel<4, 0, 1, 16>), grid, block, 0, st, p);
// ... 59 lines not shown
    GemmP p = {};
    p.A = x; p.B = wpacked; p.bias = bias; p.C = y;
    p.M = Bn * H * W; p.N = Cout; p.K = KH * KW * Cin;
    p.sbk = Cout; p.sbn = 1; p.scm = ldy; p.scn = 1;
    p.alpha = 1.f; p.beta = beta; p.act = act;
    fill_conv(p, H, W, Cin, KH, KW, xsn, xsh, xsw, xsc);
    set_split(p, splitk, ws);
    int rc = try_conv_fast(p, st);
    if (rc == 0) return p.splitk > 1 ? finish_splitk(p, 1, 0, 0, st) : 0;
    if (rc > 0) return rc;
    rc = launch_gemm<3, 16>(p, 1, true, false, st);
    if (rc) return rc;
    if (p.splitk > 1) return finish_splitk(p, 1, 0, 0, st);
    return 0;
}

TATT_API int tatt_conv2d_fwd_partials(const float* x, long xsn, long xsh, long xsw, long xsc, const float* wpacked, int Bn, int H,
                                      int W, int Cin, int Cout, int KH, int KW, int splitk, float* ws, int* splits, hipStream_t st) {
    if (!ws || !splits) return 1;
    GemmP p = {};
    p.A = x; p.B = wpacked; p.bias = nullptr; p.C = ws;
    p.M = Bn * H * W; p.N = Cout; p.K = KH * KW * Cin;
    p.sbk = Cout; p.sbn = 1; p.scm = Cout; p.scn = 1;
    p.alpha = 1.f; p.beta = 0.f; p.act = ACT_NONE;
    fill_conv(p, H, W, Cin, KH, KW, xsn, xsh, xsw, xsc);
    set_split(p, splitk, ws);
    *splits = p.splitk;
    int rc = try_conv_fast(p, st);
    if (rc >= 0) return rc;
    return launch_gemm<3, 16>(p, 1, true, false, st);
}

TATT_API int tatt_conv2d_wgrad(const float* x, long xsn, long xsh, long xsw, long xsc, const float* dy,
                               long lddy, float* dw_oihw, int Bn, int H, int W, int Cin, int Cout, int KH,
                               int KW, float beta, int splitk, float* ws, hipStream_t st) {
    GemmP p = {};
    p.A = x; p.B = dy; p.bias = nullptr; p.C = dw_oihw;
    p.M = KH * KW * Cin; p.N = Cout; p.K = Bn * H * W;
    p.sbk = lddy; p.sbn = 1; p.scm = Cout; p.scn = 1;
    p.alpha = 1.f; p.beta = beta; p.act = ACT_NONE;
    fill_conv(p, H, W, Cin, KH, KW, xsn, xsh, xsw, xsc);
    set_split(p, splitk < 2 ? 2 : splitk, ws);
    if (p.splitk < 2) { p.splitk = 2; p.chunks_per_split = cdiv(cdiv(p.K, KC), 2); }
    int rc = try_wgrad_fast(p, st);
    if (rc < 0) rc = launch_gemm<4, 16>(p, 1, false, false, st);
    if (rc) return rc;
    return finish_splitk(p, 1, Cin, KH * KW, st);
}

#define TOEPLITZ9_WORDS (9 * 4 * 2 * 6 * 64 * 4)
__device__ __forceinline__ float toeplitz9(const float* __restrict__ w, int idx, int mode) {
    const int u = idx & 3, lane = (idx >> 2) & 63;
    int r = idx >> 8;
    const int f = r % 6; r /= 6;
    const int kh = r & 1; r >>= 1;
    const int c = r & 3, ky = r >> 2;
    const int cqi = f / 3, d = f - 3 * cqi;
    const int ci = 16 * c + 4 * (kh + 2 * cqi) + (lane >> 4), nn = lane & 15;
    const int j = nn >> 2, o = nn & 3, kx = 4 * d + u - j;
    if (kx < 0 || kx >= 9) return 0.f;
    return mode == 8 ? w[(((long)o * 64 + ci) * 9 + ky) * 9 + kx] : w[(((long)ci * 4 + o) * 9 + (8 - ky)) * 9 + (8 - kx)];
}
static inline long repack_total(int Cout, int Cin, int KH, int KW, int mode) {
    return (mode == 8 || mode == 9 || mode == 12 || mode == 13) ? (long)TOEPLITZ9_WORDS : (long)Cout * Cin * KH * KW;
}
typedef __bf16 rp_bf16x2 __attribute__((ext_vector_type(2)));
typedef float rp_f32x2 __attribute__((ext_vector_type(2)));
__device__ __forceinline__ float repack_sb(const float* __restrict__ w, long idx, int Cout, int Cin, int mode) {
    const int e2 = (int)(idx & 3), lane = (int)((idx >> 2) & 63), hl = (int)((idx >> 8) & 1);
    long r = idx >> 9;
    const int ks = (int)(r % 18); r /= 18;
    const int nblk = (mode == 10 ? Cout : Cin) / 16;
    const int blk = (int)(r % nblk), chunk = (int)(r / nblk);
    const int tap = ks >> 1, half = ks & 1;
    const int o = 16 * blk + (lane & 15), i = 64 * chunk + 32 * half + 8 * (lane >> 4) + 2 * e2;
    rp_f32x2 v;
#pragma unroll
    for (int u = 0; u < 2; ++u) v[u] = mode == 10 ? w[((long)o * Cin + (i + u)) * 9 + tap] : w[((long)(i + u) * Cin + o) * 9 + (8 - tap)];
    const rp_bf16x2 hi = __builtin_convertvector(v, rp_bf16x2);
    const rp_bf16x2 lo = __builtin_convertvector(v - __builtin_convertvector(hi, rp_f32x2), rp_bf16x2);
    return __builtin_bit_cast(float, hl ? lo : hi);
}
__device__ __forceinline__ float repack_sb32(const float* __restrict__ w, long idx, int Cout, int Cin, int mode) {
    const int e2 = (int)(idx & 3), lane = (int)((idx >> 2) & 63);
    long r = idx >> 8;
    const int F = (int)(r % 72); r /= 72;
    const int nblk = (mode == 14 ? Cout : Cin) / 32;
    const int blk = (int)(r % nblk), chunk = (int)(r / nblk);
    const int hl = F & 1, sstep = (F >> 1) & 1, kh = (F >> 2) & 1, tap = F >> 3;
    const int o = 32 * blk + (lane & 31), i = 64 * chunk + 32 * kh + 16 * sstep + 8 * (lane >> 5) + 2 * e2;
    rp_f32x2 v;
#pragma unroll
    for (int u = 0; u < 2; ++u) v[u] = mode == 14 ? w[((long)o * Cin + (i + u)) * 9 + tap] : w[((long)(i + u) * Cin + o) * 9 + (8 - tap)];
    const rp_bf16x2 hi = __builtin_convertvector(v, rp_bf16x2);
    const rp_bf16x2 lo = __builtin_convertvector(v - __builtin_convertvector(hi, rp_f32x2), rp_bf16x2);
    return __builtin_bit_cast(float, hl ? lo : hi);
}
__device__ __forceinline__ float toeplitz9_sb(const float* __restrict__ w, int idx, int mode) {
    const int e2 = idx & 3, lane = (idx >> 2) & 63, hl = (idx >> 8) & 1;
    int r = idx >> 9;
    const int pair = r % 6; r /= 6;
    const int c = r & 3, ky = r >> 2;
    const int nn = lane & 15, kq = lane >> 4;
    const int j = nn >> 2, o = nn & 3, kx = 2 * pair + (kq >> 1) - j, ci = 16 * c + 8 * (kq & 1) + 2 * e2;
    rp_f32x2 v = (rp_f32x2){0.f, 0.f};
    if (kx >= 0 && kx < 9) {
#pragma unroll
        for (int u = 0; u < 2; ++u)
            v[u] = mode == 12 ? w[(((long)o * 64 + ci + u) * 9 + ky) * 9 + kx] : w[(((long)(ci + u) * 4 + o) * 9 + (8 - ky)) * 9 + (8 - kx)];
    }
    const rp_bf16x2 hi = __builtin_convertvector(v, rp_bf16x2);
    const rp_bf16x2 lo = __builtin_convertvector(v - __builtin_convertvector(hi, rp_f32x2), rp_bf16x2);
    return __builtin_bit_cast(float, hl ? lo : hi);
}
__global__ void repack_weight_kernel(const float* __restrict__ w, float* __restrict__ out, int Cout, int Cin,
                                     int KH, int KW, int mode) {
    int idx = blockIdx.x * blockDim.x + threadIdx.x;
    if (mode >= 14) {
        if (idx < Cout * Cin * 9) out[idx] = repack_sb32(w, idx, Cout, Cin, mode);
        return;
    }
    if (mode >= 12) {
        if (idx < TOEPLITZ9_WORDS) out[idx] = toeplitz9_sb(w, idx, mode);
        return;
    }
    if (mode >= 10) {
        if (idx < Cout * Cin * 9) out[idx] = repack_sb(w, idx, Cout, Cin, mode);
        return;
    }
    if (mode >= 8) {
        if (idx < TOEPLITZ9_WORDS) out[idx] = toeplitz9(w, idx, mode);
        return;
    }
    int total = Cout * Cin * KH * KW;
    if (idx >= total) return;
    int T = KH * KW;
    if (mode == 0) {
        int co = idx % Cout; int r = idx / Cout; int ci = r % Cin; int tap = r / Cin;
        out[idx] = w[((long)co * Cin + ci) * T + tap];
    } else if (mode == 1) {
        int ci = idx % Cin; int r = idx / Cin; int co = r % Cout; int tap = r / Cout;
        out[idx] = w[((long)co * Cin + ci) * T + (T - 1 - tap)];
    } else if (mode == 2) {
        int ci = idx % Cin; int r = idx / Cin; int co = r % Cout; int tap = r / Cout;
        out[idx] = w[((long)co * Cin + ci) * T + tap];
    } else if (mode == 3) {
        int co = idx % Cout; int r = idx / Cout; int ci = r % Cin; int tap = r / Cin;
        out[idx] = w[((long)co * Cin + ci) * T + (T - 1 - tap)];
    } else {
        const int u = idx & 3, lane = (idx >> 2) & 63;
        const int q6 = (idx >> 8) % 36, blk = idx / (36 * 256);
        const int tap6 = q6 >> 2, g6 = q6 & 3;
        const int o6 = blk * 16 + (lane & 15), i6 = 16 * g6 + 4 * (lane >> 4) + u;
        if (mode == 6) out[idx] = w[((long)o6 * Cin + i6) * T + tap6];
        else out[idx] = w[((long)i6 * Cin + o6) * T + (T - 1 - tap6)];
    }
}
TATT_API int tatt_repack_words(int Cout, int Cin, int KH, int KW, int mode) {
    if (mode == 4 || mode == 5 || mode < 0 || mode > 15) return -1;
    return (int)repack_total(Cout, Cin, KH, KW, mode);
}
TATT_API int tatt_repack_conv_weight(const float* w_oihw, float* out, int Cout, int Cin, int KH, int KW,
                                     int mode, hipStream_t st) {
    const bool fwd9 = mode == 8 || mode == 12, dgrad9 = mode == 9 || mode == 13;
    if ((fwd9 || dgrad9) && !(KH == 9 && KW == 9 && ((fwd9 && Cout == 4 && Cin == 64) || (dgrad9 && Cout == 64 && Cin == 4)))) return 1;
    if ((mode == 10 || mode == 11 || mode == 14 || mode == 15) && !(KH == 3 && KW == 3 && Cout % 64 == 0 && Cin % 64 == 0)) return 1;
    if (mode == 4 || mode == 5 || mode < 0 || mode > 15) return 1;
    long total = repack_total(Cout, Cin, KH, KW, mode);
    hipLaunchKernelGGL(repack_weight_kernel, dim3(cdiv(total, 256)), dim3(256), 0, st, w_oihw, out, Cout, Cin,
                       KH, KW, mode);
    return LAUNCH_CHECK();
}

#define REPACK_MAX 96
struct RepackEntry { const float* w; float* out; int Cout, Cin, KH, KW, mode, block0; };
struct RepackTable { RepackEntry e[REPACK_MAX]; int n; };
__global__ void repack_batch_kernel(RepackTable t) {
    int k = 0;
    while (k + 1 < t.n && (int)blockIdx.x >= t.e[k + 1].block0) ++k;
    const RepackEntry& e = t.e[k];
    const int idx = ((int)blockIdx.x - e.block0) * blockDim.x + threadIdx.x;
    if (e.mode >= 14) {
        if (idx < e.Cout * e.Cin * 9) e.out[idx] = repack_sb32(e.w, idx, e.Cout, e.Cin, e.mode);
        return;
    }
    if (e.mode >= 12) {
        if (idx < TOEPLITZ9_WORDS) e.out[idx] = toeplitz9_sb(e.w, idx, e.mode);
        return;
    }
    if (e.mode >= 10) {
        if (idx < e.Cout * e.Cin * 9) e.out[idx] = repack_sb(e.w, idx, e.Cout, e.Cin, e.mode);
        return;
    }
    if (e.mode >= 8) {
        if (idx < TOEPLITZ9_WORDS) e.out[idx] = toeplitz9(e.w, idx, e.mode);
        return;
    }
    const int total = e.Cout * e.Cin * e.KH * e.KW;
    if (idx >= total) return;
    const int T = e.KH * e.KW, Cout = e.Cout, Cin = e.Cin;
    const float* w = e.w;
    float v;
    if (e.mode == 0) { int co = idx % Cout; int r = idx / Cout; int ci = r % Cin; int tap = r / Cin; v = w[((long)co * Cin + ci) * T + tap]; }
    else if (e.mode == 1) { int ci = idx % Cin; int r = idx / Cin; int co = r % Cout; int tap = r / Cout; v = w[((long)co * Cin + ci) * T + (T - 1 - tap)]; }
    else if (e.mode == 2) { int ci = idx % Cin; int r = idx / Cin; int co = r % Cout; int tap = r / Cout; v = w[((long)co * Cin + ci) * T + tap]; }
    else if (e.mode == 3) { int co = idx % Cout; int r = idx / Cout; int ci = r % Cin; int tap = r / Cin; v = w[((long)co * Cin + ci) * T + (T - 1 - tap)]; }
    else {
        const int u = idx & 3, lane = (idx >> 2) & 63;
        const int q6 = (idx >> 8) % 36, blk = idx / (36 * 256);
        const int tap6 = q6 >> 2, g6 = q6 & 3;
        const int o6 = blk * 16 + (lane & 15), i6 = 16 * g6 + 4 * (lane >> 4) + u;
        v = e.mode == 6 ? w[((long)o6 * Cin + i6) * T + tap6] : w[((long)i6 * Cin + o6) * T + (T - 1 - tap6)];
    }
    e.out[idx] = v;
}
TATT_API int tatt_repack_conv_weight_batch(const float* const* ws, float* const* outs, const int* dims, int n, hipStream_t st) {
    if (n <= 0) return 0;
    for (int base = 0; base < n; base += REPACK_MAX) {
        RepackTable t;
        t.n = n - base < REPACK_MAX ? n - base : REPACK_MAX;
        int blocks = 0;
        for (int k = 0; k < t.n; ++k) {
            const int* d = dims + (long)(base + k) * 5;
            t.e[k] = {ws[base + k], outs[base + k], d[0], d[1], d[2], d[3], d[4], blocks};
            blocks += cdiv(repack_total(d[0], d[1], d[2], d[3], d[4]), 256);
        }
        hipLaunchKernelGGL(repack_batch_kernel, dim3(blocks), dim3(256), 0, st, t);
    }
    return LAUNCH_CHECK();
}

TATT_API int tatt_splitk_reduce(const float* partial, float* C, int M, int N, int S, int remap_cin, int remap_taps,
                                float beta, float* vec, int vec_len, hipStream_t st) {
    ReduceArgs a = {partial, C, nullptr, vec, (long)N, 1L, 0L, 0L, M, N, S, 1, 1.f, beta, (int)ACT_NONE, remap_cin, remap_taps, 0,
                    vec ? vec_len : 0};
    return reduce_submit(a, st);
}
```

tatt_amd/functional.py:

```python
from __future__ import annotations

import math
from typing import Optional

import weakref

import torch
from torch.autograd import Function

from . import ops
from .ops import ACT_NONE, ACT_RELU, ACT_MISH, ACT_TANH

_SEEDS = {}
_CUR_SEED = {}


def seed_tensor(device) -> torch.Tensor:
    key = str(device)
    if key not in _SEEDS:
        _SEEDS[key] = torch.tensor([0x1234ABCD5678EF01 & 0x7FFFFFFFFFFFFFFF], dtype=torch.int64, device=device)
    return _SEEDS[key]


def set_seed(device, value: int):
# ... 901 lines not shown
        return ga + gb


def fork2(x):
    return Fork2Fn.apply(x) if (x.requires_grad and torch.is_grad_enabled()) else (x, x)


class AddRowBcastFn(Function):

    @staticmethod
    def forward(ctx, a, b):
        return ops.add_rowbcast(a, b, b.shape[0])

    @staticmethod
    def backward(ctx, dy):
        return dy, None


class ScaleFn(Function):
    @staticmethod
    def forward(ctx, a, s):
        ctx.s = s
        return ops.axpby(a, None, s, 0.0)

    @staticmethod
    def backward(ctx, dy):
        return ops.axpby(_c(dy), None, ctx.s, 0.0), None


class MeanOf2Fn(Function):
    @staticmethod
    def forward(ctx, a, b):
        return ops.axpby(a, b, 0.5, 0.5)

    @staticmethod
    def backward(ctx, dy):
        h = ops.axpby(_c(dy), None, 0.5, 0.0)
        return h, h


class ActFn(Function):

    @staticmethod
    def forward(ctx, x, act):
        y = ops.act_fwd(x, act)
        ctx.save_for_backward(y)
        ctx.act = act
        return y

    @staticmethod
    def backward(ctx, dy):
        (y,) = ctx.saved_tensors
        return ops.act_bwd(y, _c(dy), ctx.act, True), None


class PReLUFn(Function):
    @staticmethod
    def forward(ctx, x, alpha):
        ctx.save_for_backward(x, alpha)
        return ops.prelu_fwd(x, alpha)

    @staticmethod
    def backward(ctx, dy):
        x, alpha = ctx.saved_tensors
        dx, da = ops.prelu_bwd(x, _c(dy), alpha)
        return dx, da.reshape(alpha.shape)


def prelu(x, alpha):
    return PReLUFn.apply(_c(x), alpha)


class PixelShuffleActFn(Function):
    @staticmethod
    def forward(ctx, x, act):
        ctx.save_for_backward(x)
        ctx.act = act
        return ops.pixel_shuffle_fwd(x, act)

    @staticmethod
    def backward(ctx, dy):
        (x,) = ctx.saved_tensors
        return ops.pixel_shuffle_bwd(x, _c(dy), ctx.act), None


class MaxPoolFn(Function):

    @staticmethod
    def forward(ctx, x, kh, kw, sh, sw, ph, pw):
        ctx.save_for_backward(x)
        ctx.k = (kh, kw, sh, sw, ph, pw)
        return ops.maxpool_fwd(x, *ctx.k)

    @staticmethod
    def backward(ctx, dy):
        (x,) = ctx.saved_tensors
        return (ops.maxpool_bwd(x, _c(dy), *ctx.k),) + (None,) * 6


def max_pool(x, kh, kw, sh=None, sw=None, ph=0, pw=0):
    return MaxPoolFn.apply(x, kh, kw, sh or kh, sw or kw, ph, pw)


class Permute4dFn(Function):

    @staticmethod
    def forward(ctx, x, perm):
        ctx.perm = perm
        return ops.to_contiguous(x.permute(*perm))

    @staticmethod
    def backward(ctx, dy):
        inv = [0] * 4
        for i, p in enumerate(ctx.perm):
            inv[p] = i
        return ops.to_contiguous(_c(dy).permute(*inv)), None


class LayerNormFn(Function):

    @staticmethod
    def forward(ctx, a, b, gamma, beta, eps, mode, p, site):
        C = a.shape[-1]
        ctx.p, ctx.site = float(p), site
        ctx.seed = current_seed(a.device) if p > 0.0 else None
        y, stats = ops.ln_fwd(a.reshape(-1, C), None if b is None else b.reshape(-1, C), gamma, beta, eps, mode, ctx.p, ctx.seed, site)
        ctx.save_for_backward(a, b, stats, gamma)
        ctx.eps, ctx.mode = eps, mode
        return y.reshape(a.shape)

    @staticmethod
    def backward(ctx, dy):
        a, b, stats, gamma = ctx.saved_tensors
        C = a.shape[-1]
        dx, db2, dg, db = ops.ln_bwd(a.reshape(-1, C), None if b is None else b.reshape(-1, C), _c(dy).reshape(-1, C), stats,
                                     gamma, ctx.eps, ctx.mode, ctx.p, ctx.seed, ctx.site)
        return dx.reshape(a.shape), (db2.reshape(a.shape) if b is not None else None), dg, db, None, None, None, None


def layer_norm(a, b, ln, p=0.0, training=False, site=0):
    p = p if (training and b is not None) else 0.0
    return LayerNormFn.apply(_c(a), None if b is None else _c(b), ln.weight, ln.bias, ln.eps, 0, p, site)


class DropoutFn(Function):
    @staticmethod
    def forward(ctx, x, p, site):
        ctx.p, ctx.site = p, site
        ctx.seed = current_seed(x.device)
        return ops.dropout(x, p, ctx.seed, site)

    @staticmethod
    def backward(ctx, dy):
        return ops.dropout(_c(dy), ctx.p, ctx.seed, ctx.site), None, None


def dropout(x, p, training, site):
    if not training or p <= 0.0:
        return x
    return DropoutFn.apply(_c(x), p, site)


class AttnCoreFn(Function):
    @staticmethod
    def forward(ctx, Q, K, V, pdrop, site):
        seed = current_seed(Q.device)
# ... 1049 lines not shown
```

tatt_amd/infer.py:

```python
from __future__ import annotations

import ctypes
import weakref
from typing import Iterable, Optional, Sequence

import torch

from . import functional as Fh
from . import ops
from ._lib import LIB
from .ops import ACT_MISH, ACT_RELU, ACT_TANH
from .io import ALPHABET, LABEL_CAP, str_filt

LSTM_CHAIN = True
LSTM_SYNC = []
LABEL_RING = 4
CTC_T = 26
D2A = "-" + ALPHABET
LABEL_FOREIGN = 64
KINDS = ("sr", "lr", "hr")
HIST = LABEL_CAP + 1


def keep_mask(voc_type: str = "lower") -> list:
# ... 225 lines not shown
                self._folds["b7"] = _Fold(b7[0], b7[1])
            self._crnn_folds = {id(m): _crnn_folds(m) for m in (prior, recognizer) if m is not None}
        self._keep = torch.tensor(keep_mask(voc_type), dtype=torch.int32, device=self.device)
        self.psnr_sum = torch.zeros((), device=self.device)
        self.ssim_sum = torch.zeros((), device=self.device)
        self.correct = torch.zeros(3, dtype=torch.int32, device=self.device)
        self.full_metrics = bool(full_metrics)
        self.psnr_lr_sum = torch.zeros((), device=self.device)
        self.ssim_lr_sum = torch.zeros((), device=self.device)
        self.ned_stats = torch.zeros(3, HIST + 2, dtype=torch.int32, device=self.device)
        self.records = None
        self.graph = None
        self._syncs, self._sync_i = [], 0
        self._sources = [t for m in (generator, prior, recognizer) if m is not None
                         for t in list(m.parameters()) + list(m.buffers())]
        self._seen = self._snapshot()

    def _snapshot(self):
        return tuple(t._version for t in self._sources), tuple(t.data_ptr() for t in self._sources)

    def _all_folds(self):
        out = [f for pair in self._folds.values() for f in (pair if isinstance(pair, tuple) else (pair,))]
        return out + [f for d in self._crnn_folds.values() for f in d.values()]

    def _repack(self, force):
        repack_filters([f.w for f in self._all_folds()], (self.gen, self.prior, self.rec), force)

    def refresh(self, force: bool = True):
        with torch.no_grad():
            for f in self._all_folds():
                f.run()
            self._repack(force)
        self._seen = (self._snapshot()[0], self._seen[1])

    def _check_weights(self):
        snap = self._snapshot()
        if snap == self._seen:
            return
        if snap[1] != self._seen[1]:
            with torch.no_grad():
                for f in self._all_folds():
                    f.run()
            self.graph = None
            self._seen = snap
            return
        self.refresh(force=False)

    def _sync(self, ref):
        if self._sync_i == len(self._syncs):
            self._syncs.append(_lstm_sync(ref))
        s = self._syncs[self._sync_i]
        self._sync_i += 1
        return s

    def _crnn(self, crnn, img):
        return crnn_eval(crnn, self._crnn_folds[id(crnn)], img, self._sync)

    def _generator(self, x, tp):
        from .tsrn import _gru_block, _nchw, _query_pos, _tp_interpreter
        m = self.gen
        k = m.srb_nums
        qpos = _query_pos(m.infoGen, x.shape[0], x.shape[2], x.shape[3]) if self.is_tatt else None
        if k > 0:
            Fh.gru_precompose([g for i in range(k) for g in (getattr(m, "block%d" % (i + 2)).gru1, getattr(m, "block%d" % (i + 2)).gru2)])
        xin = x.permute(0, 2, 3, 1)
        c1 = m.block1[0]
        b1 = Fh.prelu(Fh.conv2d(xin, c1.weight, c1.bias), m.block1[1].weight)
        tp_map = pr_weights = None
        if self.is_tatt:
            tp_map, pr_weights = _tp_interpreter(b1, tp.float(), m.infoGen, False, qpos, None)
        h = b1
        for i in range(k):
            blk = getattr(m, "block%d" % (i + 2))
            f1, f2 = self._folds["srb%d" % i]
            r = Fh.conv2d(h, f1.w, f1.b, ACT_MISH)
            r = Fh.conv2d(r, f2.w, f2.b)
            r = _gru_block(r, blk.gru1, True, x_cat=tp_map)
            h = _gru_block(Fh.add(h, r), blk.gru2, False)
        f7 = self._folds["b7"]
        h = Fh.conv2d(h, f7.w, f7.b)
        b8 = getattr(m, "block%d" % (k + 3))
        u = Fh.add(b1, h)
        for up in list(b8)[:-1]:
            u = Fh.PixelShuffleActFn.apply(Fh.conv2d(u, up.conv.weight, up.conv.bias), ACT_MISH)
        last = b8[len(b8) - 1]
        sr = Fh.ActFn.apply(Fh.conv2d(u, last.weight, last.bias), ACT_TANH)
        Fh.gru_precompose_done()
        return _nchw(sr), pr_weights

    def _forward(self):
        from .crnn import parse_crnn_data, text_prior
        self._sync_i = 0
        lr, hr, tp = self._lr, self._hr, self._tp
        prior = None
        if self.prior is not None:
            prior = text_prior(self._crnn(self.prior, parse_crnn_data(lr)))
            tp = prior
        if self.fold_gen:
            sr, pr_weights = self._generator(lr, tp)
        else:
            sr, pr_weights = self.gen(lr), None
        if hr is not None:
            from .losses import SSIM
            from .train import calculate_psnr
            self.psnr_sum += calculate_psnr(sr[:, :3], hr[:, :3])
            self.ssim_sum += SSIM()(sr[:, :3], hr[:, :3])
            if self.full_metrics:
                from .crnn import bicubic_resize
                up = bicubic_resize(lr[:, :3], hr.shape[-2:])
                self.psnr_lr_sum += calculate_psnr(up, hr[:, :3])
                self.ssim_lr_sum += SSIM()(up, hr[:, :3])
        if self.rec is not None and self._labels is not None:
            from .crnn import parse_crnn_data
            imgs = {"sr": sr, "lr": lr, "hr": hr}
            self._logits = {}
            for name in self.accuracy_on:
                if imgs[name] is None:
                    continue
                logits = self._crnn(self.rec, parse_crnn_data(imgs[name][:, :3].contiguous()))
                if logits.shape[0] != CTC_T:
                    raise RuntimeError("recogniser output has %d steps, the label buffers %d" % (logits.shape[0], CTC_T))
                self._logits[name] = logits
                k = KINDS.index(name)
                if self.full_metrics:
                    ctc_greedy_score(logits, self._keep, self._labels[0], self._labels[1], self.correct[k:], self.ned_stats[k],
                                     self.records[k])
                else:
                    ctc_greedy_match(logits, self._keep, self._labels[0], self._labels[1], self.correct[k:])
        return sr, pr_weights, prior

    def _stage_inputs(self, lr, hr, labels, text_prior):
        self._lr.copy_(lr)
        if hr is not None:
            self._hr.copy_(hr)
        if text_prior is not None:
            self._tp.copy_(text_prior)
        if labels is not None and self._labels is not None:
            codes, lens = (encode_labels_full if self.full_metrics else encode_labels)(labels, self.voc_type)
            k = self._ring_i % LABEL_RING
            self._ring_i += 1
            host, ev = self._lab_host[k], self._lab_events[k]
            if ev is not None:
                ev.synchronize()
            n = self.B * self._lab_w
            host[:n].copy_(torch.tensor(codes, dtype=torch.int32).reshape(-1))
            host[n:].copy_(torch.tensor(lens, dtype=torch.int32))
            self._lab_dev.copy_(host, non_blocking=True)
            ev = self._lab_events[k] = ev if ev is not None else torch.cuda.Event()
            ev.record()

    def _build(self, lr, hr, labels, text_prior):
        dev = self.device
        self._lr = torch.empty_like(lr, memory_format=torch.contiguous_format)
        self._hr = None if hr is None else torch.empty_like(hr, memory_format=torch.contiguous_format)
        self._tp = None
        if self.is_tatt and self.prior is None:
            self._tp = torch.zeros(1, 37, 1, 26, device=dev) if text_prior is None else torch.empty_like(text_prior)
        self._labels = None
        if labels is not None and self.rec is not None:
            self._lab_w = LABEL_CAP if self.full_metrics else CTC_T
            n = self.B * self._lab_w
            self._lab_dev = torch.full((n + self.B,), -1, dtype=torch.int32, device=dev)
            self._labels = (self._lab_dev[:n].view(self.B, self._lab_w), self._lab_dev[n:])
            if self.full_metrics:
                self.records = torch.full((3, self.B, CTC_T + 3), -1, dtype=torch.int32, device=dev)
            self._lab_host = [torch.empty(n + self.B, dtype=torch.int32, pin_memory=True) for _ in range(LABEL_RING)]
            self._lab_events, self._ring_i = [None] * LABEL_RING, 0
# ... 389 lines not shown
```

tatt_amd/ops.py:

```python
from __future__ import annotations

import ctypes
import weakref
from typing import Optional

import os

import torch

from ._lib import LIB

ACT_NONE, ACT_RELU, ACT_MISH, ACT_TANH = 0, 1, 2, 3
_vp = ctypes.c_void_p


def _check_dev(t: torch.Tensor):
    if not t.is_cuda:
        raise RuntimeError("tatt_amd kernels need tensors on an AMD GPU (HIP device); got %s. "
                           "There is no CPU fallback in the product path." % t.device)
    if t.dtype != torch.float32:
        raise RuntimeError("tatt_amd kernels are fp32; got %s" % t.dtype)


def P(t: Optional[torch.Tensor]):
# ... 452 lines not shown
    return (tuple(weight_oihw.shape) == (64, 64, 3, 3) and x_bhwc.is_contiguous()
            and x_bhwc.shape[3] == 64 and _conv3_geom_ok(x_bhwc))


def conv3_bn_forward(x_bhwc, weight_oihw, bias, in_scale=None, in_shift=None, in_act=ACT_NONE, want_stats=True):
    _check_dev(x_bhwc)
    B, H, W, _ = x_bhwc.shape
    if CONV3_SB:
        slices = _conv3_sb_slices(x_bhwc, 64, 64, ACT_NONE) or [(0, B)]
        G = sum(_conv3_sb_groups(b1 - b0, H, W) for b0, b1 in slices)
        part = new(x_bhwc, G * 128, dtype=torch.float64) if want_stats else None
        return _conv3_sb(x_bhwc, weight_oihw, 10, bias, ACT_NONE, in_scale, in_shift, in_act, part), part, G
    G = min(256, B * H * W // 64)
    part = new(x_bhwc, G * 128, dtype=torch.float64) if want_stats else None
    y = new(x_bhwc, B, H, W, 64)
    call("tatt_conv3_c64_fwd_ws16_bn", P(x_bhwc), P(repack_weight(weight_oihw, 6)), P(bias), P(y), B, H, W, 64, ACT_NONE, 0.0,
         P(in_scale), P(in_shift), int(in_act), P(part), stream())
    return y, part, G


def bn_stats_finish(part, G, C, M, eps, momentum, gamma, beta, running_mean, running_var):
    mean, rstd, scale, shift = new(gamma, C), new(gamma, C), new(gamma, C), new(gamma, C)
    call("tatt_bn_stats_finish", P(part), G, C, M, float(eps), float(momentum), P(gamma), P(beta), P(mean), P(rstd),
         P(running_mean), P(running_var), P(scale), P(shift), stream())
    return mean, rstd, scale, shift


def conv2d_dgrad(dy_bhwc, weight_oihw, any_width=False):
    Cout, Cin, KH, KW = weight_oihw.shape
    if KH == 9 and KW == 9 and Cout == 64 and Cin == 4 and _conv9_mfma_ok(dy_bhwc):
        B, H, W, _ = dy_bhwc.shape
        dx = new(dy_bhwc, B, H, W, 4)
        if CONV9_SB:
            call("tatt_conv9_c64_to_c4_sb", P(dy_bhwc), P(repack_weight(weight_oihw, 13)), None, P(dx), B, H, W, stream())
        else:
            call("tatt_conv9_c64_to_c4_mfma", P(dy_bhwc), P(repack_weight(weight_oihw, 9)), None, P(dx), B, H, W, stream())
        return dx
    if _conv3_fast_ok(dy_bhwc, Cout, Cin, KH, KW, any_width):
        B, H, W, _ = dy_bhwc.shape
        if CONV3_SB and _conv3_sb_slices(dy_bhwc, Cout, Cin, ACT_NONE) is not None:
            return _conv3_sb(dy_bhwc, weight_oihw, 11, None)
        if W % 64:
            return conv_fwd(dy_bhwc, repack_weight(weight_oihw, 1), None, Cin, KH, KW)
        dx = new(dy_bhwc, B, H, W, Cin)
        if Cout == 64:
            wl = repack_weight(weight_oihw, _WS_DGRAD_MODE)
            call(_WS_ENTRY, P(dy_bhwc), P(wl), None, P(dx), B, H, W, Cin, ACT_NONE, 0.0, stream())
            return dx
        wt = repack_weight(weight_oihw, 3)
        call("tatt_conv3_c64_fwd_t", P(dy_bhwc), P(wt), None, P(dx), B, H, W, Cout, Cin, ACT_NONE, 0.0, stream())
        return dx
    return conv_fwd(dy_bhwc, repack_weight(weight_oihw, 1), None, Cin, KH, KW)


def conv_wgrad(x_bhwc, dy_bhwc, Cout, KH, KW, want_db=False, any_width=False):
    B, H, W, Cin = x_bhwc.shape
    sn, sh, sw, sc = x_bhwc.stride()
    dw = new(x_bhwc, Cout, Cin, KH, KW)
    contig = x_bhwc.is_contiguous() and dy_bhwc.is_contiguous()
    if contig and KH == 3 and KW == 3 and Cin % 64 == 0 and Cout % 64 == 0 and (W % 64 == 0 or (CONV3_WGRAD_SB and H % 4 == 0 and ((CONV3_SB_NARROW_MAPS and W % 16 == 0) or any_width))):
        slices = (_batch_slices(B, lambda nb: LIB.tatt_conv3_wgrad_sb_route(nb, H, W, Cin, Cout) != 0) if CONV3_WGRAD_SB else None) \
            or [(0, B)]
        nblk = (Cin // 64) * (Cout // 64)
        groups = []
        for b0, b1 in slices:
            nseg = (b1 - b0) * (H // 4) * ((W + 15) // 16) if W % 64 else (b1 - b0) * H * W // 64
            groups.append(min(nseg, max(1, (CONV3_WGRAD_GROUPS if nblk == 1 else 256) // nblk)))
        G = sum(groups)
        n = G * 9 * Cin * Cout
        part = _split_ws(new(x_bhwc, n + (G * Cout if want_db else 0)))
        db = new(x_bhwc, Cout) if want_db else None
        g0 = 0
        for (b0, b1), g in zip(slices, groups):
            call("tatt_conv3_c64_wgrad_partial_sb" if CONV3_WGRAD_SB else "tatt_conv3_c64_wgrad_partial", P(x_bhwc[b0:b1]), P(dy_bhwc[b0:b1]),
                 P(part[g0 * 9 * Cin * Cout:]), P(part[n + g0 * Cout:]) if want_db else None, b1 - b0, H, W, Cin, Cout, g, stream())
            g0 += g
        call("tatt_splitk_reduce", P(part), P(dw), 9 * Cin, Cout, G, Cin, 9, 0.0, P(db), Cout, stream())
        return (dw, db) if want_db else dw
    if want_db:
        return _conv_wgrad_general(x_bhwc, dy_bhwc, dw, Cout, KH, KW, contig), colsum(dy_bhwc.reshape(-1, Cout))
    return _conv_wgrad_general(x_bhwc, dy_bhwc, dw, Cout, KH, KW, contig)


CONV_WGRAD_SPLIT_CAP = 256


def _conv_wgrad_general(x_bhwc, dy_bhwc, dw, Cout, KH, KW, contig):
    B, H, W, Cin = x_bhwc.shape
    sn, sh, sw, sc = x_bhwc.stride()
    if contig and KH == 9 and KW == 9 and Cout == 4 and Cin == 64 and H % 4 == 0 and W % 64 == 0:
        G = min(B * (H // 4) * (W // 64), 256)
        part = new(x_bhwc, G * 64 * 336)
        call("tatt_conv9_c64_c4_wgrad_sb" if CONV9_SB and CONV9_SB_WGRAD else "tatt_conv9_c64_c4_wgrad", P(x_bhwc), P(dy_bhwc), P(dw), P(part), B, H, W, stream())
        return dw
    if contig and KH == 9 and KW == 9 and Cout == 64 and Cin == 4 and H % 4 == 0 and W % 64 == 0:
        G = min(B * (H // 4) * (W // 64), 256)
        part = new(x_bhwc, G * 64 * 336)
        call("tatt_conv9_c4_c64_wgrad_sb" if CONV9_SB and CONV9_SB_WGRAD else "tatt_conv9_c4_c64_wgrad", P(x_bhwc), P(dy_bhwc), P(dw), P(part), B, H, W, stream())
        return dw
    Mo, Kred = KH * KW * Cin, B * H * W
    splitk = max(2, _auto_split(Mo, Cout, Kred, cap=CONV_WGRAD_SPLIT_CAP))
    ws = _split_ws(new(x_bhwc, (splitk + 1) * Mo * Cout))
    call("tatt_conv2d_wgrad", P(x_bhwc), sn, sh, sw, sc, P(dy_bhwc), Cout, P(dw), B, H, W, Cin, Cout, KH, KW, 0.0,
         splitk, P(ws), stream())
    return dw


def bn_stats(x2, eps, momentum, running_mean, running_var):
    M, C = x2.shape
    mean, rstd = new(x2, C), new(x2, C)
    ws = new(x2, 256 * 2 * C, dtype=torch.float64)
    call("tatt_bn_stats", P(x2), x2.stride(0), M, C, eps, momentum, P(mean), P(rstd), P(running_mean), P(running_var),
         P(ws), stream())
    return mean, rstd


def bn_rstd(var, eps):
    rstd = torch.empty_like(var)
    call("tatt_bn_rstd", P(var), P(rstd), var.numel(), eps, stream())
    return rstd


def bn_apply(x2, mean, rstd, gamma, beta, act, out=None):
    M, C = x2.shape
    y = out if out is not None else new(x2, M, C)
    call("tatt_bn_apply", P(x2), x2.stride(0), P(y), y.stride(0), M, C, P(mean), P(rstd), P(gamma), P(beta), act, stream())
    return y


def bn_bwd(x2, dy2, mean, rstd, gamma, beta, act, training):
    M, C = x2.shape
    dx = new(x2, M, C)
    dgamma, dbeta, sums = new(x2, C), new(x2, C), new(x2, 2 * C)
    ws = new(x2, 256 * 2 * C, dtype=torch.float64)
    call("tatt_bn_bwd", P(x2), x2.stride(0), P(dy2), dy2.stride(0), P(dx), C, M, C, P(mean), P(rstd), P(gamma), P(beta),
         act, int(training), P(dgamma), P(dbeta), P(sums), P(ws), stream())
    return dx, dgamma, dbeta


def bn_bwd_partials(x2, dy2, mean, rstd, gamma, beta, act):
    M, C = x2.shape
    G = LIB.tatt_bn_bwd_groups(int(M))
    part = new(x2, G * 2 * C, dtype=torch.float64)
    call("tatt_bn_bwd_partials", P(x2), x2.stride(0), P(dy2), dy2.stride(0), M, C, P(mean), P(rstd), P(gamma), P(beta), int(act),
         P(part), stream())
    return part, G


def bn_bwd_finish(part, G, C, M, mean, rstd, gamma):
    dgamma, dbeta, coef = new(gamma, C), new(gamma, C), new(gamma, 3, C)
    call("tatt_bn_bwd_finish", P(part), G, C, M, P(mean), P(rstd), P(gamma), P(dgamma), P(dbeta), P(coef), stream())
    return dgamma, dbeta, coef


def bn_bwd_affine(x2, du2, coef):
    M, C = x2.shape
    dx = new(x2, M, C)
    call("tatt_bn_bwd_affine", P(x2), P(du2), P(dx), M, C, P(coef), stream())
    return dx


def conv3_dgrad_bn(du_bhwc, weight_oihw, x2_bhwc=None, coef=None, ep=None):
    _check_dev(du_bhwc)
    B, H, W, _ = du_bhwc.shape
    if LIB.tatt_conv3_sb_generation(0) != CONV3_SB_GENERATION:
        LIB.tatt_conv3_sb_generation(int(CONV3_SB_GENERATION))
# ... 400 lines not shown
```

tatt_amd/tbsrn.py:

```python
from __future__ import annotations

import copy
import math

import torch
from torch import nn

from . import functional as Fh
from . import ops
from .ops import ACT_NONE, ACT_RELU, ACT_MISH, ACT_TANH
from .tsrn import (_Holder, GruBlock, UpsampleBLock, STNHead, TPSSpatialTransformer, _stn_forward, _tps_forward,
                   _require_gpu, _nchw, _TrainPathMixin)


def positionalencoding2d(d_model, height, width):
    pe = torch.zeros(d_model, height, width)
    half = d_model // 2
    div_term = torch.exp(torch.arange(0., half, 2) * -(math.log(10000.0) / half))
    pos_w = torch.arange(0., width).unsqueeze(1)
    pos_h = torch.arange(0., height).unsqueeze(1)
    pe[0:half:2] = torch.sin(pos_w * div_term).transpose(0, 1).unsqueeze(1).repeat(1, height, 1)
    pe[1:half:2] = torch.cos(pos_w * div_term).transpose(0, 1).unsqueeze(1).repeat(1, height, 1)
    pe[half::2] = torch.sin(pos_h * div_term).transpose(0, 1).unsqueeze(2).repeat(1, 1, width)
    pe[half + 1::2] = torch.cos(pos_h * div_term).transpose(0, 1).unsqueeze(2).repeat(1, 1, width)
# ... 70 lines not shown
def _feature_enhancer(r, fe: FeatureEnhancer, training, dropout_on, site0):
    B, H, W, C = r.shape
    Pn = H * W
    drop = training and dropout_on
    x = Fh.CatPEFn.apply(r.reshape(B, Pn, C), fe.pe_tokens(H, W, r.device))
    mh = fe.multihead
    ln1, ln3 = fe.mul_layernorm1, fe.mul_layernorm3
    x = Fh.attention_ln(x, mh, ln1.a_2, ln1.b_2, ln1.eps, 1, mh.p if drop else 0.0, site0)
    x = Fh.feed_forward_ln(x, fe.pff.w_1, fe.pff.w_2, ln3.a_2, ln3.b_2, ln3.eps, 1, fe.pff.p, drop, site0 + 1)
    x = Fh.linear(x, fe.linear.weight, fe.linear.bias)
    return x.reshape(B, H, W, C)


def _srb(x, blk: RecurrentResidualBlock, training, dropout_on, site0):
    r = Fh.conv2d(x, blk.conv1.weight, blk.conv1.bias)
    r = Fh.batch_norm_act(r, blk.bn1, ACT_MISH)
    r = Fh.conv2d(r, blk.conv2.weight, blk.conv2.bias)
    r = Fh.batch_norm_act(r, blk.bn2, ACT_NONE)
    r = _feature_enhancer(r, blk.feature_enhancer, training, dropout_on, site0)
    return Fh.add(x, r)


class TBSRN(_TrainPathMixin, nn.Module):

    def __init__(self, scale_factor=2, width=128, height=32, STN=True, srb_nums=5, mask=False, hidden_units=32,
                 input_channel=3):
        super().__init__()
        self.conv = nn.Conv2d(input_channel, 3, 3, 1, 1)
        self.bn = nn.BatchNorm2d(3)
        in_planes = 4 if mask else 3
        assert math.log(scale_factor, 2) % 1 == 0
        upsample_block_num = int(math.log(scale_factor, 2))
        C = 2 * hidden_units
        self.block1 = nn.Sequential(nn.Conv2d(in_planes, C, kernel_size=9, padding=4), nn.PReLU())
        self.srb_nums = srb_nums
        for i in range(srb_nums):
            setattr(self, "block%d" % (i + 2), RecurrentResidualBlock(C))
        setattr(self, "block%d" % (srb_nums + 2), nn.Sequential(nn.Conv2d(C, C, kernel_size=3, padding=1),
                                                                  nn.BatchNorm2d(C)))
        blk = [UpsampleBLock(C, 2) for _ in range(upsample_block_num)]
        blk.append(nn.Conv2d(C, in_planes, kernel_size=9, padding=4))
        setattr(self, "block%d" % (srb_nums + 3), nn.Sequential(*blk))
        self.tps_inputsize = [height // scale_factor, width // scale_factor]
        self.stn = STN
        if self.stn:
            self.tps = TPSSpatialTransformer(tuple(self.tps_inputsize), 20, (0.05, 0.05))
            self.stn_head = STNHead(in_planes, 20, "none")
        self.dropout_on = True

    def forward(self, x):
        _require_gpu(x)
        training = self.training
        k = self.srb_nums
        cuts = self._grad_cuts if training else None
        if training:
            Fh.begin_training_forward(x.device)
        if self.stn and training:
            ctrl = _stn_forward(x, self.stn_head)
            if cuts:
                ctrl = cuts.cut("stn", ctrl)
            xin, _ = _tps_forward(x, ctrl, self.tps)
        else:
            xin = x.permute(0, 2, 3, 1)
        c1 = self.block1[0]
        b1 = Fh.prelu(Fh.conv2d(xin, c1.weight, c1.bias), self.block1[1].weight)
        b1_in = b1
        Fh.linear_prepack([l for i in range(k) for l in _fe_linears(getattr(self, "block%d" % (i + 2)).feature_enhancer)])
        if cuts:
            b1 = cuts.cut("first", b1_in)
        h = b1_in
        for i in range(k):
            if cuts:
                h = cuts.cut("first", b1_in) if i == 0 else cuts.cut("srb%d" % (i - 1), h)
            h = _srb(h, getattr(self, "block%d" % (i + 2)), training, self.dropout_on, 100 + 10 * i)
        Fh.linear_prepack_done()
        if cuts and k > 0:
            h = cuts.cut("srb%d" % (k - 1), h)
        b7 = getattr(self, "block%d" % (k + 2))
        h = Fh.conv2d(h, b7[0].weight, b7[0].bias)
        h = Fh.batch_norm_act(h, b7[1], ACT_NONE)
        b8 = getattr(self, "block%d" % (k + 3))
        u = Fh.add(b1, h)
        for m in list(b8)[:-1]:
            u = Fh.conv2d(u, m.conv.weight, m.conv.bias)
            u = Fh.PixelShuffleActFn.apply(u, ACT_MISH)
        last = b8[len(b8) - 1]
        u = Fh.conv2d(u, last.weight, last.bias)
        return _nchw(Fh.ActFn.apply(u, ACT_TANH))
```

tatt_amd/tsrn.py:

```python
from __future__ import annotations

import copy
import math

import numpy as np
import torch
from torch import nn

from . import functional as Fh
from .ops import ACT_NONE, ACT_RELU, ACT_MISH, ACT_TANH
from . import ops


def _nchw(x_nhwc):
    return x_nhwc.permute(0, 3, 1, 2)


class _Holder(nn.Module):
    def forward(self, *a, **k):
        raise RuntimeError("parameter holder: the computation runs in tatt_amd's HIP kernels")


class GruBlock(_Holder):

# ... 454 lines not shown
                                                                  nn.BatchNorm2d(C)))
        blk = [UpsampleBLock(C, 2) for _ in range(upsample_block_num)]
        blk.append(nn.Conv2d(C, in_planes, kernel_size=9, padding=4))
        setattr(self, "block%d" % (srb_nums + 3), nn.Sequential(*blk))
        self.tps_inputsize = [height // scale_factor, width // scale_factor]
        self.stn = STN
        if self.stn:
            self.tps = TPSSpatialTransformer(tuple(self.tps_inputsize), 20, (0.05, 0.05))
            self.stn_head = STNHead(in_planes, 20, "none", **stn_kw)

    def _check_hip_submodules(self):
        return self

    def _trunk_forward(self, x, text_emb, use_tp):
        _require_gpu(x)
        if x.dtype != torch.float32:
            raise RuntimeError("tatt_amd computes in fp32; got %s" % x.dtype)
        training = self.training
        k = self.srb_nums
        cuts = self._grad_cuts if training else None
        qpos = None
        pre_forked = False
        if use_tp:
            if PRECOMPOSE_ON_FORK and k > 0 and isinstance(getattr(self, "block2").gru1, GruBlock):
                Fh.FWD_FORK.run(x, lambda: Fh.gru_precompose([g for i in range(k) for g in (getattr(self, "block%d" % (i + 2)).gru1,
                                                                                         getattr(self, "block%d" % (i + 2)).gru2)]))
                pre_forked = True
            qpos = _query_pos(self.infoGen, x.shape[0], x.shape[2], x.shape[3])
        if training:
            Fh.begin_training_forward(x.device)
            self._bump_bn_counters()
        if use_tp and text_emb is None:
            text_emb = torch.zeros(1, 37, 1, 26, device=x.device)
        text_side = None
        if not pre_forked and k > 0 and isinstance(getattr(self, "block2").gru1, GruBlock):
            Fh.gru_precompose([g for i in range(k) for g in (getattr(self, "block%d" % (i + 2)).gru1,
                                                             getattr(self, "block%d" % (i + 2)).gru2)])
        if self.stn and training:
            ctrl = _stn_forward(x, self.stn_head, False)
            if cuts:
                ctrl = cuts.cut("stn", ctrl)
            Fh.stamp("fwd: stn head done", x)
            xin, _ = _tps_forward(x, ctrl, self.tps)
        else:
            xin = x.permute(0, 2, 3, 1)
        c1 = self.block1[0]
        b1 = Fh.prelu(Fh.conv2d(xin, c1.weight, c1.bias), self.block1[1].weight)
        Fh.stamp("fwd: block1 done", x)
        feats = {"1": b1}
        tp_map = pr_weights = None
        b1_trunk = b1
        if use_tp:
            Fh.FWD_FORK_B.join(x.device)
            tp_map, pr_weights = _tp_interpreter(cuts.cut("first", b1) if cuts else b1, text_emb.float(), self.infoGen, training,
                                                 qpos, text_side)
        tp_ret = tp_map
        if cuts:
            b1_trunk = cuts.cut("first", b1)
        h = b1
        for i in range(k):
            if cuts:
                h_in = cuts.cut("first", b1) if i == 0 else cuts.cut("srb%d" % (i - 1), h)
                tp_in = cuts.cut("tp", tp_map) if tp_map is not None else None
            else:
                h_in, tp_in = h, tp_map
            if i == 0:
                Fh.stamp("fwd: tp done", x)
            h = _srb(h_in, tp_in, getattr(self, "block%d" % (i + 2)))
            Fh.stamp("fwd: srb%d done" % i, x)
            feats[str(i + 2)] = h
        if cuts and k > 0:
            h = cuts.cut("srb%d" % (k - 1), h)
        b7 = getattr(self, "block%d" % (k + 2))
        if b7[1].training and ops.conv3_bn_fusable(h, b7[0].weight, b7[1]):
            y7, st7 = Fh.conv_bn(_cc(h), b7[0], b7[1])
            h = Fh.bn_apply_stats(y7, st7, b7[1], ACT_NONE)
        else:
            h = Fh.conv2d(h, b7[0].weight, b7[0].bias)
            h = Fh.batch_norm_act(h, b7[1], ACT_NONE, False)
        feats[str(k + 2)] = h
        b8 = getattr(self, "block%d" % (k + 3))
        u = Fh.add(b1_trunk, h)
        for m in list(b8)[:-1]:
            u = Fh.conv2d(u, m.conv.weight, m.conv.bias)
            u = Fh.PixelShuffleActFn.apply(u, ACT_MISH)
        last = b8[len(b8) - 1]
        u = Fh.conv2d(u, last.weight, last.bias)
        feats[str(k + 3)] = u
        sr = Fh.ActFn.apply(u, ACT_TANH)
        Fh.stamp("fwd: sr done", x)
        Fh.gru_precompose_done()
        self.block = {kk: _nchw(v) for kk, v in feats.items()}
        return _nchw(sr), tp_ret, pr_weights, b1


class TSRN(_GeneratorBase):

    def __init__(self, scale_factor=2, width=128, height=32, STN=False, srb_nums=5, mask=True, hidden_units=32):
        super().__init__()
        in_planes, C, ub = self._build_trunk(scale_factor, width, height, STN, srb_nums, mask, hidden_units, 0)
        self._build_tail(in_planes, C, ub, scale_factor, width, height, STN, {})

    def forward(self, x):
        sr, _, _, _ = self._trunk_forward(x, None, False)
        return sr


class TSRN_TL_TRANS(_GeneratorBase):

    def __init__(self, scale_factor=2, width=128, height=32, STN=False, srb_nums=5, mask=True, hidden_units=32,
                 word_vec_d=300, text_emb=37, out_text_channels=64, feature_rotate=False, rotate_train=3.):
        super().__init__()
        in_planes, C, ub = self._build_trunk(scale_factor, width, height, STN, srb_nums, mask, hidden_units,
                                             out_text_channels)
        self.infoGen = TPInterpreter(text_emb, out_text_channels,
                                     output_size=(height // scale_factor, width // scale_factor))
        self.feature_rotate = feature_rotate
        self.rotate_train = rotate_train
        self._build_tail(in_planes, C, ub, scale_factor, width, height, STN,
                         {"input_size": [height // scale_factor, width // scale_factor]})
        self.block_range = [k for k in range(2, self.srb_nums + 2)]

    def forward(self, x, text_emb=None, text_emb_gt=None, feature_arcs=None, rand_offs=None):
        sr, tp_map, pr_weights, b1 = self._trunk_forward(x, text_emb, True)
        if self.training:
            tp_nchw = _nchw(tp_map)
            ret_mid = {"pr_weights": pr_weights, "pr_weights_gt": None, "spatial_t_emb": tp_nchw,
                       "spatial_t_emb_gt": None, "in_feat": _nchw(b1), "trans_feat": tp_nchw}
            return sr, ret_mid
        return sr, pr_weights
```

Before: 11800.

## Fuse upsample conv3 with pixel-shuffle and Mish in fwd, dgrad and wgrad

Adds an UpsampleConvFn path that runs the 64->256 conv3 of the upsample block with pixel-shuffle and Mish folded into the split-bf16 conv epilogue. It writes the high-res output plus a Mish-gradient gate tensor directly. Backward multiplies dout by the gate while loading the halo for dgrad (four 64-channel sub-passes) and for wgrad, and reduces with a column-permuted split-K. This removes the intermediate 256-channel tensor and the separate pixel-shuffle passes. In exchange it stores an extra gate tensor and adds more kernel template variants.

```diff
diff --git a/include/tatt_hip.h b/include/tatt_hip.h
--- a/include/tatt_hip.h
+++ b/include/tatt_hip.h
@@ -60,6 +60,15 @@
                                     int Cin, int Cout, int G, hipStream_t st);
 int tatt_conv3_wgrad_sb_generation(int gen);
 int tatt_conv3_wgrad_sb_route(int B, int H, int W, int Cin, int Cout);
+int tatt_conv3_up_route(int B, int H, int W);
+int tatt_conv3_up_fwd_sb(const float* x, const float* wl, const float* bias, float* y, float* gate, int B, int H, int W, int Cout,
+                         int act, float beta, double* stats, hipStream_t st);
+int tatt_conv3_up_dgrad_sb(const float* dout, const float* gate, int sub, const float* wl, float* dx, int B, int H, int W,
+                           float beta, hipStream_t st);
+int tatt_conv3_up_wgrad_partial_sb(const float* x, const float* dout, const float* gate, float* part, float* pdb, int B, int H,
+                                   int W, int G, hipStream_t st);
+int tatt_splitk_reduce_cols(const float* partial, float* C, int M, int N, int S, int remap_cin, int remap_taps,
+                            float beta, float* vec, int vec_len, int colperm, hipStream_t st);
 
 int tatt_conv9_c64_to_c4(const float* x, const float* wpacked, const float* bias, float* y, int B, int H, int W,
                          int C, hipStream_t st);
diff --git a/tatt_amd/csrc/conv3.hip b/tatt_amd/csrc/conv3.hip
--- a/tatt_amd/csrc/conv3.hip
+++ b/tatt_amd/csrc/conv3.hip
@@ -345,6 +345,7 @@
     Conv3P c; int cin_total, ci0;
     const float* x2; const float* in_scale2;
     const float* ep_x; const float* ep_mean; const float* ep_rstd; const float* ep_gamma; const float* ep_beta; int ep_act;
+    float* y2; int ups;
 };
 __device__ __forceinline__ void sb_split(f32x4 v, uint2& hi, uint2& lo) {
     const bf16x2 h0 = __builtin_convertvector((f32x2){v[0], v[1]}, bf16x2), h1 = __builtin_convertvector((f32x2){v[2], v[3]}, bf16x2);
@@ -354,6 +355,11 @@
     const bf16x2 l0 = __builtin_convertvector((f32x2){r0, r1}, bf16x2), l1 = __builtin_convertvector((f32x2){r2, r3}, bf16x2);
     hi = make_uint2(u0, u1);
     lo = make_uint2(__builtin_bit_cast(unsigned, l0), __builtin_bit_cast(unsigned, l1));
+}
+__device__ __forceinline__ float sb_mul_rn(float a, float b) {
+    float r = a * b;
+    asm("" : "+v"(r));
+    return r;
 }
 template <bool IN2, bool EPBN>
 __global__ __launch_bounds__(512, 1) void conv3_c64_sb_kernel(Conv3SB q) {
@@ -802,7 +808,7 @@
         }
     }
 }
-template <int INMODE, bool EPBN>
+template <int INMODE, bool EPBN, bool UPS = false>
 __global__ __launch_bounds__(512, 2) void conv3_c64_sb4_kernel(Conv3SB q) {
     const Conv3P& p = q.c;
     extern __shared__ __attribute__((aligned(16))) unsigned smem_u[];
@@ -832,13 +838,22 @@
         const unsigned cin = min(18u, W - tw * 16 + 1);
         te = (th == 0 ? 1u : 0u) | (th == ths - 1 ? 2u : 0u) | (tw == 0 ? 4u : 0u) | (cin << 8);
     };
+    auto decode_hr = [&](unsigned tile, unsigned& orgb, unsigned& te) {
+        const unsigned tw = tile % tws; tile /= tws;
+        const unsigned th = tile % ths, n = tile / ths;
+        orgb = ((n * H + th * 4) * W * 8 + tw * 64) * 128;
+        const unsigned cin = min(18u, W - tw * 16 + 1);
+        te = (th == 0 ? 1u : 0u) | (th == ths - 1 ? 2u : 0u) | (tw == 0 ? 4u : 0u) | (cin << 8);
+    };
+    constexpr bool AFF = INMODE >= 1 && INMODE <= 3;
     if (wave >= 4) {
         const unsigned h = t - 256;
         const unsigned npix = p.B * H * W;
         const __amdgpu_buffer_rsrc_t rs_x = __builtin_amdgcn_make_buffer_rsrc(const_cast<float*>(p.x), 0, npix * q.cin_total * 4, 0x00020000);
-        const __amdgpu_buffer_rsrc_t rs_x2 = __builtin_amdgcn_make_buffer_rsrc(const_cast<float*>(INMODE == 2 ? q.x2 : p.x), 0, npix * 256, 0x00020000);
+        const __amdgpu_buffer_rsrc_t rs_x2 = __builtin_amdgcn_make_buffer_rsrc(const_cast<float*>((INMODE == 2 || INMODE == 4) ? q.x2 : p.x), 0, INMODE == 4 ? npix * q.cin_total * 4 : npix * 256, 0x00020000);
         const __amdgpu_buffer_rsrc_t rs_y = __builtin_amdgcn_make_buffer_rsrc(p.y, 0, npix * p.Cout * 4, 0x00020000);
         const __amdgpu_buffer_rsrc_t rs_e = __builtin_amdgcn_make_buffer_rsrc(const_cast<float*>(EPBN ? q.ep_x : p.y), 0, npix * (EPBN ? 64 : p.Cout) * 4, 0x00020000);
+        const __amdgpu_buffer_rsrc_t rs_g = __builtin_amdgcn_make_buffer_rsrc((UPS && q.y2) ? q.y2 : p.y, 0, npix * p.Cout * 4, 0x00020000);
         const bool in_relu = p.in_act == ACT_RELU;
         const unsigned xps = q.cin_total * 4, yps = p.Cout * 4, eps_ = EPBN ? 256u : yps;
         unsigned boff[S3_NIT], poff[S3_NIT], edge[2] = {0, 0}, colk[2] = {0, 0};
@@ -853,13 +868,36 @@
         auto outside = [&](int k, unsigned te) -> bool {
             return (((edge[k >> 2] >> (8 * (k & 3))) & (te | 8u) & 15u) != 0) || (((colk[k >> 2] >> (8 * (k & 3))) & 255u) >= (te >> 8));
         };
-        f32x4 hp[S3_NIT], hp2[S3_NIT];
+        unsigned boff4[2], poff4[2], edge4 = 0, colk4 = 0;
+#pragma unroll
+        for (int j = 0; j < 2; ++j) {
+            const unsigned pix = (h >> 2) + 64 * j, r = pix / S2_HW, c = pix - r * S2_HW;
+            boff4[j] = (unsigned)(((int)r - 1) * (int)(W * 1024) + ((int)c - 1) * 512) + ((q.ci0 >> 2) + 4 * (h & 3)) * 4;
+            poff4[j] = r * S3_RP + c * SB_PW + 8 * (h & 3);
+            edge4 |= ((r == 0 ? 1u : 0u) | (r == 5 ? 2u : 0u) | (c == 0 ? 4u : 0u) | (pix >= S2_NPX ? 8u : 0u)) << (8 * j);
+            colk4 |= c << (8 * j);
+        }
+        auto outside4 = [&](int j, unsigned te) -> bool {
+            return (((edge4 >> (8 * j)) & (te | 8u) & 15u) != 0) || (((colk4 >> (8 * j)) & 255u) >= (te >> 8));
+        };
+        f32x4 hp[INMODE == 4 ? 8 : S3_NIT], hp2[INMODE == 4 ? 8 : S3_NIT];
         auto halo_issue = [&](unsigned tile, bool valid) {
             unsigned org, te;
-            decode(tile, org, te);
+            if (INMODE == 4) decode_hr(tile, org, te); else decode(tile, org, te);
 #if S2_DEBUG
             if (s2_wrep & 4) valid = false;
 #endif
+            if (INMODE == 4) {
+#pragma unroll
+                for (int j = 0; j < 2; ++j)
+#pragma unroll
+                    for (int sp = 0; sp < 4; ++sp) {
+                        const unsigned a = (org + boff4[j] + ((sp >> 1) * 2 * W + (sp & 1)) * 256) | (outside4(j, te) ? S2_OOB : (valid ? 0u : S2_OOB));
+                        hp[4 * j + sp] = s2_ld(rs_x, a);
+                        hp2[4 * j + sp] = s2_ld(rs_x2, a);
+                    }
+                return;
+            }
 #pragma unroll
             for (int k = 0; k < S3_NIT; ++k) {
                 const unsigned a = (org * xps + boff[k]) | (outside(k, te) ? S2_OOB : (valid ? 0u : S2_OOB));
@@ -870,8 +908,26 @@
         auto halo_put = [&](unsigned* img, unsigned tile) {
             unsigned org, te;
             decode(tile, org, te);
+            if (INMODE == 4) {
+#pragma unroll
+                for (int j = 0; j < 2; ++j)
+                    if (j == 0 || h < (S2_NPX - 64) * 4) {
+#pragma unroll
+                        for (int e = 0; e < 4; ++e) {
+                            f32x4 v;
+#pragma unroll
+                            for (int sp = 0; sp < 4; ++sp) v[sp] = sb_mul_rn(hp[4 * j + sp][e], hp2[4 * j + sp][e]);
+                            uint2 hi, lo;
+                            sb_split(v, hi, lo);
+                            unsigned* d = img + poff4[j] + 2 * e;
+                            *reinterpret_cast<uint2*>(d) = hi;
+                            *reinterpret_cast<uint2*>(d + S3_IMG) = lo;
+                        }
+                    }
+                return;
+            }
             f32x4 isc, ish, isc2;
-            if (INMODE != 0) { isc = *reinterpret_cast<const f32x4*>(&cst[0][4 * (h & 15)]); ish = *reinterpret_cast<const f32x4*>(&cst[1][4 * (h & 15)]); }
+            if (AFF) { isc = *reinterpret_cast<const f32x4*>(&cst[0][4 * (h & 15)]); ish = *reinterpret_cast<const f32x4*>(&cst[1][4 * (h & 15)]); }
             if (INMODE == 2) isc2 = *reinterpret_cast<const f32x4*>(&cst[2][4 * (h & 15)]);
 #pragma unroll
             for (int k = 0; k < S3_NIT; ++k) {
@@ -890,7 +946,7 @@
                         v[e] = in_relu ? fmaxf(u, 0.f) : u;
                     }
                 }
-                if (INMODE != 0) {
+                if (AFF) {
 #pragma unroll
                     for (int e = 0; e < 4; ++e) v[e] = ok ? v[e] : 0.f;
                 }
@@ -905,8 +961,10 @@
         };
         halo_issue(pt, true);
         if (h < 64) {
+            if (UPS) cbias[h] = p.bias ? p.bias[4 * h + cb] : 0.f;
+            else
             cbias[h] = p.bias ? p.bias[cb * 64 + h] : 0.f;
-            if (INMODE != 0) { cst[0][h] = p.in_scale[h]; cst[1][h] = p.in_shift[h]; }
+            if (AFF) { cst[0][h] = p.in_scale[h]; cst[1][h] = p.in_shift[h]; }
             if (INMODE == 2) cst[2][h] = q.in_scale2[h];
             if (EPBN) { cst[3][h] = q.ep_mean[h]; cst[4][h] = q.ep_rstd[h]; cst[5][h] = q.ep_gamma[h]; cst[6][h] = q.ep_beta[h]; }
         }
@@ -919,6 +977,7 @@
         const unsigned ecol = h >> 4, ec4 = 4 * (h & 15);
         f32x4 epx[S3_NEP], st_s = (f32x4){0.f, 0.f, 0.f, 0.f}, st_q = st_s;
         auto epi_request = [&](unsigned tile) {
+            if (UPS) return;
             unsigned org, te;
             decode(tile, org, te);
             const bool in_map = ecol + 1 < (te >> 8);
@@ -928,7 +987,7 @@
         };
         auto epilogue = [&](unsigned tile, unsigned xb) {
             unsigned org, te;
-            decode(tile, org, te);
+            if (UPS) decode_hr(tile, org, te); else decode(tile, org, te);
             const f32x4 bj = *reinterpret_cast<const f32x4*>(&cbias[ec4]);
             const bool in_map = ecol + 1 < (te >> 8);
             f32x4 ep_mu, ep_rs, ep_g, ep_b;
@@ -941,6 +1000,19 @@
                 const unsigned* X = XCH + xb * S2_XCH + ((h >> 4) + 16 * e) * S2_XP + ec4;
                 const f32x4 v0 = *reinterpret_cast<const f32x4*>(X), v1 = *reinterpret_cast<const f32x4*>(X + 64 * S2_XP);
                 f32x4 v;
+                if (UPS) {
+                    f32x4 g;
+#pragma unroll
+                    for (int r = 0; r < 4; ++r) {
+                        const float u = (v0[r] + v1[r]) + bj[r];
+                        v[r] = mish_f(u);
+                        g[r] = mish_grad_f(u);
+                    }
+                    const unsigned a = org + (e * W * 8 + ecol * 4) * 128 + (((cb >> 1) * 2 * W + (cb & 1)) * 64 + ec4) * 4;
+                    __builtin_amdgcn_raw_buffer_store_b128(__builtin_bit_cast(u32x4_s2, v), rs_y, a | (in_map ? 0u : S2_OOB), 0, 0);
+                    __builtin_amdgcn_raw_buffer_store_b128(__builtin_bit_cast(u32x4_s2, g), rs_g, a | ((in_map && q.y2) ? 0u : S2_OOB), 0, 0);
+                    continue;
+                }
 #pragma unroll
                 for (int r = 0; r < 4; ++r) {
                     v[r] = (v0[r] + v1[r]) + bj[r];
@@ -1060,13 +1132,13 @@
     if (gen == 1 || gen == 3 || gen == 4) conv3_sb_generation = gen;
     return old;
 }
-template <int INMODE, bool EPBN>
+template <int INMODE, bool EPBN, bool UPS = false>
 static void conv3_sb4_go(const Conv3SB& q, dim3 grid, hipStream_t st) {
     static TattPerDevice attr_once;
     tatt_per_device(attr_once, [&] {
-        (void)hipFuncSetAttribute(reinterpret_cast<const void*>(conv3_c64_sb4_kernel<INMODE, EPBN>), hipFuncAttributeMaxDynamicSharedMemorySize, S3_LDS);
+        (void)hipFuncSetAttribute(reinterpret_cast<const void*>(conv3_c64_sb4_kernel<INMODE, EPBN, UPS>), hipFuncAttributeMaxDynamicSharedMemorySize, S3_LDS);
     });
-    hipLaunchKernelGGL((conv3_c64_sb4_kernel<INMODE, EPBN>), grid, dim3(512), S3_LDS, st, q);
+    hipLaunchKernelGGL((conv3_c64_sb4_kernel<INMODE, EPBN, UPS>), grid, dim3(512), S3_LDS, st, q);
 }
 template <int INMODE, bool EPBN>
 static void conv3_sb3_go(const Conv3SB& q, dim3 grid, hipStream_t st) {
@@ -1099,6 +1171,11 @@
         const dim3 grid(per * cob);
         const bool ep = q.ep_x != nullptr;
         const int inmode = q.x2 ? 2 : (p.in_scale ? (p.in_act == ACT_MISH ? 1 : 3) : 0);
+        if (q.ups) {
+            if (pick != 4) return 5;
+            if (q.ups == 1) conv3_sb4_go<0, false, true>(q, grid, st); else conv3_sb4_go<4, false>(q, grid, st);
+            return LAUNCH_CHECK();
+        }
         if (pick == 4) {
             if (inmode == 2) { if (ep) conv3_sb4_go<2, true>(q, grid, st); else conv3_sb4_go<2, false>(q, grid, st); }
             else if (inmode == 1) { if (ep) conv3_sb4_go<1, true>(q, grid, st); else conv3_sb4_go<1, false>(q, grid, st); }
@@ -1115,6 +1192,7 @@
         }
         return LAUNCH_CHECK();
     }
+    if (q.ups) return 5;
     if (p.W % C3_PX) return 1;
     static TattPerDevice attr_once;
     tatt_per_device(attr_once, [&] {
@@ -1141,7 +1219,7 @@
     if (stats && (Cout != 64 || act != ACT_NONE || beta != 0.f)) return 2;
     if (in_scale && (!in_shift || in_act == ACT_TANH)) return 3;
     Conv3SB q = {{x, wl, bias, y, B, H, W, 64, Cout, act, beta, in_scale, in_shift, in_act, stats}, cin_total, ci0,
-                 nullptr, nullptr, nullptr, nullptr, nullptr, nullptr, nullptr, 0};
+                 nullptr, nullptr, nullptr, nullptr, nullptr, nullptr, nullptr, 0, nullptr, 0};
     return conv3_sb_launch(q, st);
 }
 TATT_API int tatt_conv3_c64_dgrad_bn_sb(const float* x, const float* x2, const float* in_scale, const float* in_scale2,
@@ -1152,7 +1230,25 @@
     if (ep_x && (!ep_mean || !ep_rstd || !ep_gamma || !ep_beta || !stats)) return 3;
     if (!ep_x && stats) return 4;
     Conv3SB q = {{x, wl, nullptr, y, B, H, W, 64, 64, ACT_NONE, 0.f, x2 ? in_scale : nullptr, x2 ? in_shift : nullptr, ACT_NONE, stats}, 64, 0,
-                 x2, in_scale2, ep_x, ep_mean, ep_rstd, ep_gamma, ep_beta, ep_act};
+                 x2, in_scale2, ep_x, ep_mean, ep_rstd, ep_gamma, ep_beta, ep_act, nullptr, 0};
+    return conv3_sb_launch(q, st);
+}
+TATT_API int tatt_conv3_up_route(int B, int H, int W) {
+    return (conv3_sb_pick(B, H, W, 64, 256, ACT_NONE, ACT_NONE) == 4 && conv3_sb_pick(B, H, W, 256, 64, ACT_NONE, ACT_NONE) == 4) ? 4 : 0;
+}
+TATT_API int tatt_conv3_up_fwd_sb(const float* x, const float* wl, const float* bias, float* y, float* gate, int B, int H, int W, int Cout,
+                                  int act, float beta, double* stats, hipStream_t st) {
+    if (Cout != 256 || act != ACT_MISH) return 1;
+    if (beta != 0.f || stats) return 2;
+    Conv3SB q = {{x, wl, bias, y, B, H, W, 64, 256, ACT_NONE, 0.f, nullptr, nullptr, ACT_NONE, nullptr}, 64, 0,
+                 nullptr, nullptr, nullptr, nullptr, nullptr, nullptr, nullptr, 0, gate, 1};
+    return conv3_sb_launch(q, st);
+}
+TATT_API int tatt_conv3_up_dgrad_sb(const float* dout, const float* gate, int sub, const float* wl, float* dx, int B, int H, int W,
+                                    float beta, hipStream_t st) {
+    if (sub < 0 || sub > 3 || !gate) return 1;
+    Conv3SB q = {{dout, wl, nullptr, dx, B, H, W, 64, 64, ACT_NONE, beta, nullptr, nullptr, ACT_NONE, nullptr}, 256, 64 * sub,
+                 gate, nullptr, nullptr, nullptr, nullptr, nullptr, nullptr, 0, nullptr, 2};
     return conv3_sb_launch(q, st);
 }
 
diff --git a/tatt_amd/csrc/conv3w.hip b/tatt_amd/csrc/conv3w.hip
--- a/tatt_amd/csrc/conv3w.hip
+++ b/tatt_amd/csrc/conv3w.hip
@@ -19,6 +19,7 @@
     const float* x; const float* dy; float* part;
     int B, H, W, Cin, Cout, nseg;
     float* pdb;
+    const float* gate;
 };
 
 __device__ __forceinline__ void cw_split(const float* v, cw_bf16x8& hi, cw_bf16x8& lo) {
@@ -198,6 +199,12 @@
     *reinterpret_cast<uint2*>(dst_hi) = make_uint2(__builtin_bit_cast(unsigned, h0), __builtin_bit_cast(unsigned, h1));
     *reinterpret_cast<uint2*>(dst_hi + lo_off) = make_uint2(__builtin_bit_cast(unsigned, l0), __builtin_bit_cast(unsigned, l1));
 }
+__device__ __forceinline__ float w2_mul_rn(float a, float b) {
+    float r = a * b;
+    asm("" : "+v"(r));
+    return r;
+}
+template <bool GATE>
 __global__ __launch_bounds__(512, 2) void conv3_c64_wgrad_sb2_kernel(Conv3WSP p) {
     extern __shared__ __attribute__((aligned(16))) char w2_smem[];
     __shared__ float dbred[16][64];
@@ -214,11 +221,16 @@
         org = (n * H + th * 4) * W + tw * 16;
         te = (th == 0 ? 1u : 0u) | (th == ths - 1 ? 2u : 0u) | (tw == 0 ? 4u : 0u) | (min(18u, W - tw * 16 + 1) << 8);
     };
+    auto origin_hr = [&](unsigned tile) -> unsigned {
+        const unsigned tw = tile % tws; tile /= tws;
+        return (tile * 4 * W * 8 + tw * 64) * 128;
+    };
     if (wave >= 4) {
         const unsigned h = t - 256, c4 = h & 15;
         const unsigned npix = p.B * H * W;
         const __amdgpu_buffer_rsrc_t rs_x = __builtin_amdgcn_make_buffer_rsrc(const_cast<float*>(p.x), 0, npix * p.Cin * 4, 0x00020000);
         const __amdgpu_buffer_rsrc_t rs_d = __builtin_amdgcn_make_buffer_rsrc(const_cast<float*>(p.dy), 0, npix * p.Cout * 4, 0x00020000);
+        const __amdgpu_buffer_rsrc_t rs_g = __builtin_amdgcn_make_buffer_rsrc(const_cast<float*>(GATE ? p.gate : p.dy), 0, npix * p.Cout * 4, 0x00020000);
         const unsigned xps = p.Cin * 4, dps = p.Cout * 4;
         unsigned xoff[7], xput[7], edge[2] = {0, 0}, colk[2] = {0, 0}, doff[4], dput[4];
 #pragma unroll
@@ -232,10 +244,12 @@
 #pragma unroll
         for (int k = 0; k < 4; ++k) {
             const unsigned pix = (h >> 4) + 16 * k;
+            if (GATE) doff[k] = (k * W * 8 + (h >> 4) * 4) * 128 + (((cob >> 1) * 2 * W + (cob & 1)) * 64 + 4 * c4) * 4;
+            else
             doff[k] = (k * W + (h >> 4)) * dps + (co0 + 4 * c4) * 4;
             dput[k] = 2 * W2_XIMG + pix * W2_PB + 8 * c4;
         }
-        f32x4 hx[7], hd[4], dbacc = (f32x4){0.f, 0.f, 0.f, 0.f};
+        f32x4 hx[7], hd[4], hg[4], dbacc = (f32x4){0.f, 0.f, 0.f, 0.f};
         auto issue = [&](unsigned tile, bool valid) {
             unsigned org, te;
             decode(tile, org, te);
@@ -246,16 +260,25 @@
                 hx[k] = __builtin_bit_cast(f32x4, __builtin_amdgcn_raw_buffer_load_b128(rs_x, (org * xps + xoff[k]) | (out ? W2_OOB : inv), 0, 0));
             }
             const unsigned dinv = ((h >> 4) + 1 < (te >> 8)) ? inv : W2_OOB;
-#pragma unroll
-            for (int k = 0; k < 4; ++k)
-                hd[k] = __builtin_bit_cast(f32x4, __builtin_amdgcn_raw_buffer_load_b128(rs_d, (org * dps + doff[k]) | dinv, 0, 0));
+            const unsigned dorg = GATE ? origin_hr(tile) : org * dps;
+#pragma unroll
+            for (int k = 0; k < 4; ++k) {
+                hd[k] = __builtin_bit_cast(f32x4, __builtin_amdgcn_raw_buffer_load_b128(rs_d, (dorg + doff[k]) | dinv, 0, 0));
+                if (GATE) hg[k] = __builtin_bit_cast(f32x4, __builtin_amdgcn_raw_buffer_load_b128(rs_g, (dorg + doff[k]) | dinv, 0, 0));
+            }
         };
         auto put = [&](char* buf) {
 #pragma unroll
             for (int k = 0; k < 7; ++k)
                 if (k < 6 || h < 1728 - 6 * 256) w2_split_put(buf + xput[k], W2_XIMG, hx[k]);
 #pragma unroll
-            for (int k = 0; k < 4; ++k) { w2_split_put(buf + dput[k], W2_DIMG, hd[k]); dbacc += hd[k]; }
+            for (int k = 0; k < 4; ++k) {
+                if (GATE) {
+#pragma unroll
+                    for (int e = 0; e < 4; ++e) hd[k][e] = w2_mul_rn(hd[k][e], hg[k][e]);
+                }
+                w2_split_put(buf + dput[k], W2_DIMG, hd[k]); dbacc += hd[k];
+            }
         };
         if (s_beg < s_end) {
             issue(s_beg, true);
@@ -354,16 +377,16 @@
     if (pick == 0) return 1;
     if (pick == 2) {
         const int ntile = B * (H / 4) * ((W + 15) / 16);
-        Conv3WSP p2 = {x, dy, part, B, H, W, Cin, Cout, ntile, pdb};
+        Conv3WSP p2 = {x, dy, part, B, H, W, Cin, Cout, ntile, pdb, nullptr};
         static TattPerDevice attr2_once;
         tatt_per_device(attr2_once, [&] {
-            (void)hipFuncSetAttribute(reinterpret_cast<const void*>(conv3_c64_wgrad_sb2_kernel), hipFuncAttributeMaxDynamicSharedMemorySize, W2_LDS);
+            (void)hipFuncSetAttribute(reinterpret_cast<const void*>(conv3_c64_wgrad_sb2_kernel<false>), hipFuncAttributeMaxDynamicSharedMemorySize, W2_LDS);
         });
-        hipLaunchKernelGGL(conv3_c64_wgrad_sb2_kernel, dim3(G, (Cin / 64) * (Cout / 64)), dim3(512), W2_LDS, st, p2);
+        hipLaunchKernelGGL(conv3_c64_wgrad_sb2_kernel<false>, dim3(G, (Cin / 64) * (Cout / 64)), dim3(512), W2_LDS, st, p2);
         return LAUNCH_CHECK();
     }
     const int nseg = B * H * (W / CW_PX);
-    Conv3WSP p = {x, dy, part, B, H, W, Cin, Cout, nseg, pdb};
+    Conv3WSP p = {x, dy, part, B, H, W, Cin, Cout, nseg, pdb, nullptr};
     static TattPerDevice attr_once;
     tatt_per_device(attr_once, [&] {
         (void)hipFuncSetAttribute(reinterpret_cast<const void*>(conv3_c64_wgrad_sb_kernel), hipFuncAttributeMaxDynamicSharedMemorySize, CW_LDS);
@@ -371,3 +394,16 @@
     hipLaunchKernelGGL(conv3_c64_wgrad_sb_kernel, dim3(G, (Cin / 64) * (Cout / 64)), dim3(512), CW_LDS, st, p);
     return LAUNCH_CHECK();
 }
+
+TATT_API int tatt_conv3_up_wgrad_partial_sb(const float* x, const float* dout, const float* gate, float* part, float* pdb, int B, int H,
+                                            int W, int G, hipStream_t st) {
+    if (conv3_wgrad_sb_pick(B, H, W, 64, 256) != 2 || !gate) return 1;
+    const int ntile = B * (H / 4) * ((W + 15) / 16);
+    Conv3WSP p2 = {x, dout, part, B, H, W, 64, 256, ntile, pdb, gate};
+    static TattPerDevice attr_once;
+    tatt_per_device(attr_once, [&] {
+        (void)hipFuncSetAttribute(reinterpret_cast<const void*>(conv3_c64_wgrad_sb2_kernel<true>), hipFuncAttributeMaxDynamicSharedMemorySize, W2_LDS);
+    });
+    hipLaunchKernelGGL(conv3_c64_wgrad_sb2_kernel<true>, dim3(G, 4), dim3(512), W2_LDS, st, p2);
+    return LAUNCH_CHECK();
+}
diff --git a/tatt_amd/csrc/gemm.hip b/tatt_amd/csrc/gemm.hip
--- a/tatt_amd/csrc/gemm.hip
+++ b/tatt_amd/csrc/gemm.hip
@@ -581,6 +581,7 @@
     float alpha, beta;
     int act, remap_cin, remap_taps, block0;
     int RM;
+    int colperm;
 };
 __device__ __forceinline__ void splitk_reduce_body(const ReduceArgs& a, long block) {
     __shared__ float sh[4][64];
@@ -598,7 +599,10 @@
         if (i2 < rm) for (int k = ty; k < S; k += 4) r += partial[(long)S * M * N + (long)k * rm + i2];
         sh[ty][tx] = r;
         __syncthreads();
-        if (ty == 0 && i2 < rm) a.rowsum[i2] = a.alpha * ((sh[0][tx] + sh[1][tx]) + (sh[2][tx] + sh[3][tx]));
+        if (ty == 0 && i2 < rm) {
+            const long o2 = a.colperm > 0 ? (long)a.colperm * (i2 % (rm / a.colperm)) + i2 / (rm / a.colperm) : i2;
+            a.rowsum[o2] = a.alpha * ((sh[0][tx] + sh[1][tx]) + (sh[2][tx] + sh[3][tx]));
+        }
         return;
     }
     const bool ok = idx < total;
@@ -629,7 +633,8 @@
     long off;
     if (a.remap_cin > 0) {
         int tap = i / a.remap_cin, ci = i - tap * a.remap_cin;
-        off = ((long)j * a.remap_cin + ci) * a.remap_taps + tap;
+        const int jo = a.colperm > 0 ? a.colperm * (j % (N / a.colperm)) + j / (N / a.colperm) : j;
+        off = ((long)jo * a.remap_cin + ci) * a.remap_taps + tap;
     } else {
         off = (long)z * a.bsC + i * a.scm + j * a.scn;
     }
@@ -855,6 +860,8 @@
     return __builtin_bit_cast(float, hl ? lo : hi);
 }
 __device__ __forceinline__ float repack_sb32(const float* __restrict__ w, long idx, int Cout, int Cin, int mode) {
+    const bool subpx = mode == 16;
+    mode -= subpx ? 2 : 0;
     const int e2 = (int)(idx & 3), lane = (int)((idx >> 2) & 63);
     long r = idx >> 8;
     const int F = (int)(r % 72); r /= 72;
@@ -864,7 +871,10 @@
     const int o = 32 * blk + (lane & 31), i = 64 * chunk + 32 * kh + 16 * sstep + 8 * (lane >> 5) + 2 * e2;
     rp_f32x2 v;
 #pragma unroll
-    for (int u = 0; u < 2; ++u) v[u] = mode == 14 ? w[((long)o * Cin + (i + u)) * 9 + tap] : w[((long)(i + u) * Cin + o) * 9 + (8 - tap)];
+    for (int u = 0; u < 2; ++u) {
+        const int oo = subpx ? 4 * (o & 63) + (o >> 6) : o;
+        v[u] = mode == 14 ? w[((long)oo * Cin + (i + u)) * 9 + tap] : w[((long)(i + u) * Cin + o) * 9 + (8 - tap)];
+    }
     const rp_bf16x2 hi = __builtin_convertvector(v, rp_bf16x2);
     const rp_bf16x2 lo = __builtin_convertvector(v - __builtin_convertvector(hi, rp_f32x2), rp_bf16x2);
     return __builtin_bit_cast(float, hl ? lo : hi);
@@ -930,7 +940,8 @@
     }
 }
 TATT_API int tatt_repack_words(int Cout, int Cin, int KH, int KW, int mode) {
-    if (mode == 4 || mode == 5 || mode < 0 || mode > 15) return -1;
+    if (mode == 4 || mode == 5 || mode < 0 || mode > 16) return -1;
+    if (mode == 16 && !(KH == 3 && KW == 3 && Cout == 256 && Cin % 64 == 0)) return -1;
     return (int)repack_total(Cout, Cin, KH, KW, mode);
 }
 TATT_API int tatt_repack_conv_weight(const float* w_oihw, float* out, int Cout, int Cin, int KH, int KW,
@@ -938,7 +949,8 @@
     const bool fwd9 = mode == 8 || mode == 12, dgrad9 = mode == 9 || mode == 13;
     if ((fwd9 || dgrad9) && !(KH == 9 && KW == 9 && ((fwd9 && Cout == 4 && Cin == 64) || (dgrad9 && Cout == 64 && Cin == 4)))) return 1;
     if ((mode == 10 || mode == 11 || mode == 14 || mode == 15) && !(KH == 3 && KW == 3 && Cout % 64 == 0 && Cin % 64 == 0)) return 1;
-    if (mode == 4 || mode == 5 || mode < 0 || mode > 15) return 1;
+    if (mode == 16 && !(KH == 3 && KW == 3 && Cout == 256 && Cin % 64 == 0)) return 1;
+    if (mode == 4 || mode == 5 || mode < 0 || mode > 16) return 1;
     long total = repack_total(Cout, Cin, KH, KW, mode);
     hipLaunchKernelGGL(repack_weight_kernel, dim3(cdiv(total, 256)), dim3(256), 0, st, w_oihw, out, Cout, Cin,
                        KH, KW, mode);
@@ -1006,6 +1018,13 @@
 TATT_API int tatt_splitk_reduce(const float* partial, float* C, int M, int N, int S, int remap_cin, int remap_taps,
                                 float beta, float* vec, int vec_len, hipStream_t st) {
     ReduceArgs a = {partial, C, nullptr, vec, (long)N, 1L, 0L, 0L, M, N, S, 1, 1.f, beta, (int)ACT_NONE, remap_cin, remap_taps, 0,
-                    vec ? vec_len : 0};
+                    vec ? vec_len : 0, 0};
     return reduce_submit(a, st);
 }
+TATT_API int tatt_splitk_reduce_cols(const float* partial, float* C, int M, int N, int S, int remap_cin, int remap_taps,
+                                     float beta, float* vec, int vec_len, int colperm, hipStream_t st) {
+    if (colperm <= 0 || remap_cin <= 0 || N % colperm || (vec && vec_len != N)) return 1;
+    ReduceArgs a = {partial, C, nullptr, vec, (long)N, 1L, 0L, 0L, M, N, S, 1, 1.f, beta, (int)ACT_NONE, remap_cin, remap_taps, 0,
+                    vec ? vec_len : 0, colperm};
+    return reduce_submit(a, st);
+}
diff --git a/tatt_amd/functional.py b/tatt_amd/functional.py
--- a/tatt_amd/functional.py
+++ b/tatt_amd/functional.py
@@ -1007,6 +1007,67 @@
     def backward(ctx, dy):
         (x,) = ctx.saved_tensors
         return ops.pixel_shuffle_bwd(x, _c(dy), ctx.act), None
+
+
+UPSAMPLE_FOLD = True
+
+
+class UpsampleConvFn(Function):
+
+    @staticmethod
+    def forward(ctx, x, weight, bias, act, any_width=False):
+        ctx.fold = bool(UPSAMPLE_FOLD and ops.conv3_up_route(x, weight, act, any_width))
+        ctx.act, ctx.any_width, ctx.has_bias, ctx.leaves = act, any_width, bias is not None, (weight, bias)
+        if ctx.fold:
+            y, gate = ops.conv3_up_forward(x, weight, bias, any(ctx.needs_input_grad))
+            ctx.save_for_backward(x, weight, gate)
+            return y
+        u = ops.conv2d_forward(x, weight, bias, ACT_NONE, any_width)
+        ctx.save_for_backward(x, weight, u)
+        return ops.pixel_shuffle_fwd(u, act)
+
+    @staticmethod
+    def backward(ctx, dy):
+        x, weight, aux = ctx.saved_tensors
+        Cout, Cin, KH, KW = weight.shape
+        dy = _c(dy)
+        want_dw, want_db = ctx.needs_input_grad[1], ctx.has_bias and ctx.needs_input_grad[2]
+        aw = ctx.any_width
+        wleaf, bleaf = ctx.leaves
+        split = want_dw and want_db and SIDE.enabled and (SIDE.due_of.get(id(wleaf)) != SIDE.due_of.get(id(bleaf))
+                                                          or (id(wleaf) in SIDE.immediate) != (id(bleaf) in SIDE.immediate))
+        if ctx.fold:
+            gate = aux
+            dx = ops.conv3_up_dgrad(dy, gate, weight) if ctx.needs_input_grad[0] else None
+
+            def param_grads():
+                dw, db = ops.conv3_up_wgrad(x, dy, gate, want_db)
+                return (dw if want_dw else None), db
+            if split:
+                (dw,) = SIDE.submit((wleaf,), lambda: (ops.conv3_up_wgrad(x, dy, gate, False)[0],), x, dy, gate)
+                (db,) = SIDE.submit((bleaf,), lambda: (ops.conv3_up_wgrad(x, dy, gate, True)[1],), x, dy, gate)
+                return dx, dw, db, None, None
+            dw, db = SIDE.submit(ctx.leaves, param_grads, x, dy, gate)
+            return dx, dw, db, None, None
+        du = ops.pixel_shuffle_bwd(aux, dy, ctx.act)
+        dx = ops.conv2d_dgrad(du, weight, aw) if ctx.needs_input_grad[0] else None
+
+        def param_grads2():
+            if want_dw and want_db:
+                return ops.conv_wgrad(x, du, Cout, KH, KW, want_db=True, any_width=aw)
+            dw = ops.conv_wgrad(x, du, Cout, KH, KW, any_width=aw) if want_dw else None
+            db = ops.colsum(du.reshape(-1, Cout)) if want_db else None
+            return dw, db
+        if split:
+            (dw,) = SIDE.submit((wleaf,), lambda: (ops.conv_wgrad(x, du, Cout, KH, KW, any_width=aw),), x, du)
+            (db,) = SIDE.submit((bleaf,), lambda: (ops.colsum(du.reshape(-1, Cout)),), du)
+            return dx, dw, db, None, None
+        dw, db = SIDE.submit(ctx.leaves, param_grads2, x, du)
+        return dx, dw, db, None, None
+
+
+def upsample_conv(x, weight, bias, act=ACT_MISH, any_width=False):
+    return UpsampleConvFn.apply(x, weight, bias, act, any_width)
 
 
 class MaxPoolFn(Function):
diff --git a/tatt_amd/infer.py b/tatt_amd/infer.py
--- a/tatt_amd/infer.py
+++ b/tatt_amd/infer.py
@@ -331,7 +331,7 @@
         b8 = getattr(m, "block%d" % (k + 3))
         u = Fh.add(b1, h)
         for up in list(b8)[:-1]:
-            u = Fh.PixelShuffleActFn.apply(Fh.conv2d(u, up.conv.weight, up.conv.bias), ACT_MISH)
+            u = Fh.UpsampleConvFn.apply(u, up.conv.weight, up.conv.bias, ACT_MISH)
         last = b8[len(b8) - 1]
         sr = Fh.ActFn.apply(Fh.conv2d(u, last.weight, last.bias), ACT_TANH)
         Fh.gru_precompose_done()
diff --git a/tatt_amd/ops.py b/tatt_amd/ops.py
--- a/tatt_amd/ops.py
+++ b/tatt_amd/ops.py
@@ -558,6 +558,54 @@
     return _conv_wgrad_general(x_bhwc, dy_bhwc, dw, Cout, KH, KW, contig)
 
 
+def conv3_up_route(x_bhwc, weight_oihw, act, any_width=False):
+    if not (x_bhwc.is_cuda and x_bhwc.dtype == torch.float32 and x_bhwc.dim() == 4 and x_bhwc.is_contiguous()):
+        return 0
+    if tuple(weight_oihw.shape) != (256, 64, 3, 3) or x_bhwc.shape[3] != 64 or act != ACT_MISH or not weight_oihw.is_contiguous():
+        return 0
+    if not (CONV3_SB and CONV3_WGRAD_SB and CONV3_SB_GENERATION == 4 and _conv3_geom_ok(x_bhwc, any_width)):
+        return 0
+    B, H, W, _ = x_bhwc.shape
+    if LIB.tatt_conv3_sb_generation(0) != CONV3_SB_GENERATION:
+        LIB.tatt_conv3_sb_generation(int(CONV3_SB_GENERATION))
+    if LIB.tatt_conv3_up_route(B, H, W) != 4 or LIB.tatt_conv3_wgrad_sb_route(B, H, W, 64, 256) != 2:
+        return 0
+    return 4
+
+
+def conv3_up_forward(x_bhwc, weight_oihw, bias, want_gate):
+    _check_dev(x_bhwc)
+    B, H, W, _ = x_bhwc.shape
+    y = new(x_bhwc, B, 2 * H, 2 * W, 64)
+    gate = torch.empty_like(y) if want_gate else None
+    call("tatt_conv3_up_fwd_sb", P(x_bhwc), P(repack_weight(weight_oihw, 16)), P(bias), P(y), P(gate), B, H, W, 256, ACT_MISH, 0.0, None,
+         stream())
+    return y, gate
+
+
+def conv3_up_dgrad(dout_hr, gate_hr, weight_oihw):
+    B, H2, W2, _ = dout_hr.shape
+    H, W = H2 // 2, W2 // 2
+    wl = repack_weight(weight_oihw, 15)
+    dx = new(dout_hr, B, H, W, 64)
+    for q in range(4):
+        call("tatt_conv3_up_dgrad_sb", P(dout_hr), P(gate_hr), q, P(wl[q * 64 * 576:]), P(dx), B, H, W, 0.0 if q == 0 else 1.0, stream())
+    return dx
+
+
+def conv3_up_wgrad(x_bhwc, dout_hr, gate_hr, want_db=True):
+    B, H, W, _ = x_bhwc.shape
+    nseg = B * (H // 4) * ((W + 15) // 16)
+    G = min(nseg, 256 // 4)
+    n = G * 9 * 64 * 256
+    part = _split_ws(new(x_bhwc, n + (G * 256 if want_db else 0)))
+    dw = new(x_bhwc, 256, 64, 3, 3)
+    db = new(x_bhwc, 256) if want_db else None
+    call("tatt_conv3_up_wgrad_partial_sb", P(x_bhwc), P(dout_hr), P(gate_hr), P(part), P(part[n:]) if want_db else None, B, H, W, G, stream())
+    call("tatt_splitk_reduce_cols", P(part), P(dw), 9 * 64, 256, G, 64, 9, 0.0, P(db), 256, 4, stream())
+    return dw, db
+
+
 CONV_WGRAD_SPLIT_CAP = 256
 
 
diff --git a/tatt_amd/tbsrn.py b/tatt_amd/tbsrn.py
--- a/tatt_amd/tbsrn.py
+++ b/tatt_amd/tbsrn.py
@@ -176,8 +176,7 @@
         b8 = getattr(self, "block%d" % (k + 3))
         u = Fh.add(b1, h)
         for m in list(b8)[:-1]:
-            u = Fh.conv2d(u, m.conv.weight, m.conv.bias)
-            u = Fh.PixelShuffleActFn.apply(u, ACT_MISH)
+            u = Fh.UpsampleConvFn.apply(u, m.conv.weight, m.conv.bias, ACT_MISH)
         last = b8[len(b8) - 1]
         u = Fh.conv2d(u, last.weight, last.bias)
         return _nchw(Fh.ActFn.apply(u, ACT_TANH))
diff --git a/tatt_amd/tsrn.py b/tatt_amd/tsrn.py
--- a/tatt_amd/tsrn.py
+++ b/tatt_amd/tsrn.py
@@ -560,8 +560,7 @@
         b8 = getattr(self, "block%d" % (k + 3))
         u = Fh.add(b1_trunk, h)
         for m in list(b8)[:-1]:
-            u = Fh.conv2d(u, m.conv.weight, m.conv.bias)
-            u = Fh.PixelShuffleActFn.apply(u, ACT_MISH)
+            u = Fh.UpsampleConvFn.apply(u, m.conv.weight, m.conv.bias, ACT_MISH)
         last = b8[len(b8) - 1]
         u = Fh.conv2d(u, last.weight, last.bias)
         feats[str(k + 3)] = u
```

Result: no change. 11900 (median of 6 runs) (+0.9%).
